# andimarafioti/faster-qwen3-tts

Hardware: AMD Instinct MI355X
Metric: real-time factor (audio s / wall s), Qwen3-TTS-12Hz-0.6B voice-clone streaming chunk_size=8; p50 TTFA in ttfa_ms_p50 (higher is better)
Workload: dtype bf16

## Files before the change

### faster-qwen3-tts_amd/csrc/fq3_api.hip

```cpp
#define FQ3_SKINNY_EXTERN
#include "fq3_ctx.h"
#include "sampler.cuh"
#include "sampler_wave.cuh"
#include "skinny_gemm.cuh"

#include <cstdio>
#include <cstdlib>
#include <cstring>
#include <map>
#include <string>
#include <type_traits>
#include <vector>

using namespace fq3;

static thread_local std::string g_err;
static int fail(int code, const std::string& m) { g_err = m; return code; }
int fq3_fail_(int code, const std::string& m) { return fail(code, m); }
#define HIPCHK(x) do { hipError_t e_ = (x); if (e_ != hipSuccess) return fail(FQ3_EHIP, std::string(#x) + ": " + hipGetErrorString(e_)); } while (0)

extern "C" const char* fq3_last_error(void) { return g_err.c_str(); }
extern "C" void fq3_set_error_(const char* msg) { g_err = msg ? msg : ""; }
extern "C" int fq3_abi_version(void) { return FQ3_ABI_VERSION; }

static int dmalloc(fq3_ctx* c, void** p, size_t bytes, bool zero = true) {
    HIPCHK(hipMalloc(p, bytes));
    if (zero) HIPCHK(hipMemset(*p, 0, bytes));
    c->allocs.push_back(*p);
    return 0;
}
int fq3_dmalloc_(fq3_ctx* c, void** p, size_t bytes) { return dmalloc(c, p, bytes, false); }

static bool dims_ok(const fq3_stack_dims& d) {
    return d.head_dim == kHeadDim && d.hidden % 8 == 0 && d.inter % 8 == 0 && d.n_heads % d.n_kv_heads == 0 &&
           (d.n_heads / d.n_kv_heads == 1 || d.n_heads / d.n_kv_heads == 2 || d.n_heads / d.n_kv_heads == 4) &&
           d.vocab <= kMaxVocab && d.vocab % 8 == 0 && d.hidden <= 2048 && d.inter <= 6144 && d.n_heads * kHeadDim <= 6144 && d.n_layers >= 1;
}

static int cfg_check(const fq3_config* cfg) {
    if (cfg->dtype != FQ3_BF16 && cfg->dtype != FQ3_F32) return fail(FQ3_EINVAL, "dtype must be FQ3_BF16 or FQ3_F32");
    if (!dims_ok(cfg->talker) || !dims_ok(cfg->predictor))
        return fail(FQ3_EUNSUPPORTED, "unsupported dims (need head_dim 128, GQA ratio 1/2/4, vocab <= 4096 and a multiple of 8, "
                                      "hidden <= 2048 and intermediate <= 6144, both multiples of 8)");
    if (cfg->num_code_groups < 2 || cfg->num_code_groups > 64) return fail(FQ3_EINVAL, "num_code_groups");
    if (cfg->max_seq_len < 8) return fail(FQ3_EINVAL, "max_seq_len");
    return 0;
}

static void pool_free_(fq3_kv_pool* p) {
    for (void* q : p->k) if (q) (void)hipFree(q);
    for (void* q : p->v) if (q) (void)hipFree(q);
    delete p;
}

static int pool_create_(const fq3_config* cfg, int n_blocks, fq3_kv_pool** out) {
    if (n_blocks < 1) return fail(FQ3_EINVAL, "fq3_kv_pool_create: n_blocks must be positive");
    fq3_kv_pool* p = new fq3_kv_pool();
    p->dtype = cfg->dtype; p->esz = cfg->dtype == FQ3_BF16 ? 2 : 4;
    p->n_layers = cfg->talker.n_layers; p->n_kv = cfg->talker.n_kv_heads; p->n_blocks = n_blocks;
    p->blk_elems = (size_t)p->n_kv * kKeysPerTile * kHeadDim;
    p->k.assign(p->n_layers, nullptr); p->v.assign(p->n_layers, nullptr);
    const size_t bytes = (size_t)n_blocks * p->blk_elems * p->esz;
    for (int i = 0; i < p->n_layers; ++i) {
        if (hipMalloc(&p->k[i], bytes) != hipSuccess || hipMalloc(&p->v[i], bytes) != hipSuccess ||
            hipMemset(p->k[i], 0, bytes) != hipSuccess || hipMemset(p->v[i], 0, bytes) != hipSuccess) {
            pool_free_(p);
            return fail(FQ3_EHIP, "fq3_kv_pool_create: allocation of " + std::to_string(2 * bytes >> 20) + " MiB per layer failed");
        }
    }
    p->free_list.resize(n_blocks);
    for (int i = 0; i < n_blocks; ++i) p->free_list[i] = n_blocks - 1 - i;
    *out = p;
    return FQ3_OK;
}

extern "C" int fq3_kv_pool_create(const fq3_config* cfg, int n_blocks, fq3_kv_pool** out) {
    if (!cfg || !out) return fail(FQ3_EINVAL, "null argument");
    if (int r = cfg_check(cfg)) return r;
    return pool_create_(cfg, n_blocks, out);
}

extern "C" int fq3_kv_pool_destroy(fq3_kv_pool* p) {
    if (!p) return FQ3_OK;
    if (p->users > 0) return fail(FQ3_ESTATE, "fq3_kv_pool_destroy: contexts are still attached");
    (void)hipDeviceSynchronize();
    pool_free_(p);
    return FQ3_OK;
}

extern "C" int fq3_kv_pool_stats(const fq3_kv_pool* p, int* n_blocks, int* n_free, int* high_water, int64_t* bytes_per_block) {
    if (!p) return fail(FQ3_EINVAL, "null pool");
    fq3_kv_pool* q = const_cast<fq3_kv_pool*>(p);
    std::lock_guard<std::mutex> lk(q->mu);
    if (n_blocks) *n_blocks = p->n_blocks;
    if (n_free) *n_free = (int)p->free_list.size();
    if (high_water) *high_water = p->in_use_high;
    if (bytes_per_block) *bytes_per_block = (int64_t)2 * p->n_layers * p->blk_elems * p->esz;
    return FQ3_OK;
}

struct KvTableVals { int v[128]; };
__global__ void kv_table_write_kernel(int* table, KvTableVals vals, int first, int count) {
    const int i = threadIdx.x;
    if (i < count) table[first + i] = vals.v[i];
}
static void table_write(fq3_ctx* c, const int* ids, int first, int count, hipStream_t s) {
    for (int o = 0; o < count; o += 128) {
        KvTableVals t{};
        const int n = std::min(128, count - o);
        for (int i = 0; i < n; ++i) t.v[i] = ids[o + i];
        hipLaunchKernelGGL(kv_table_write_kernel, dim3(1), dim3(128), 0, s, c->tk.d_table, t, first + o, n);
    }
}

static int kv_ensure(fq3_ctx* c, int n_pos, hipStream_t s, bool sync_copy);
int fq3_kv_ensure_(fq3_ctx* c, int n_pos, hipStream_t s) { return kv_ensure(c, n_pos, s, false); }
static int kv_ensure(fq3_ctx* c, int n_pos, hipStream_t s, bool sync_copy) {
    StackBufs& b = c->tk;
    int need = (std::min(n_pos, b.max_seq) + kKeysPerTile - 1) / kKeysPerTile;
    need = std::min(need, b.max_blocks);
    const int have = (int)b.blocks.size();
    if (need <= have) return 0;
    fq3_kv_pool* p = b.pool;
    {
        std::lock_guard<std::mutex> lk(p->mu);
        if ((int)p->free_list.size() < need - have) {
            char m[200];
            snprintf(m, sizeof m, "KV pool exhausted: %d more block(s) of 64 keys needed, %d free of %d", need - have, (int)p->free_list.size(), p->n_blocks);
            return fail(FQ3_ENOMEM, m);
        }
        for (int i = have; i < need; ++i) { b.blocks.push_back(p->free_list.back()); p->free_list.pop_back(); }
        p->in_use_high = std::max(p->in_use_high, p->n_blocks - (int)p->free_list.size());
    }
    if (sync_copy) HIPCHK(hipMemcpy(b.d_table + have, b.blocks.data() + have, (size_t)(need - have) * sizeof(int), hipMemcpyHostToDevice));
    else table_write(c, b.blocks.data() + have, have, need - have, s);
    return 0;
}

extern "C" int fq3_kv_release(fq3_ctx* c, int keep_positions) {
    if (!c) return fail(FQ3_EINVAL, "null ctx");
    StackBufs& b = c->tk;
    const int keep = std::max(0, std::min((int)b.blocks.size(), (keep_positions + kKeysPerTile - 1) / kKeysPerTile));
    if (keep >= (int)b.blocks.size()) return FQ3_OK;
    std::lock_guard<std::mutex> lk(b.pool->mu);
    while ((int)b.blocks.size() > keep) { b.pool->free_list.push_back(b.blocks.back()); b.blocks.pop_back(); }
    return FQ3_OK;
}

extern "C" int fq3_kv_blocks(const fq3_ctx* c) { return c ? (int)c->tk.blocks.size() : 0; }

extern "C" int fq3_kv_reserve(fq3_ctx* c, int n_positions, void* stream) {
    if (!c) return fail(FQ3_EINVAL, "null ctx");
    if (n_positions < 0) return fail(FQ3_EINVAL, "fq3_kv_reserve: negative position count");
    return fq3_kv_ensure_(c, n_positions, (hipStream_t)stream);
}

static int ctx_build(fq3_ctx* c, const fq3_config* cfg, fq3_kv_pool* pool);
static int ctx_create_(const fq3_config* cfg, fq3_kv_pool* pool, fq3_ctx** out) {
    if (!cfg || !out) return fail(FQ3_EINVAL, "null argument");
    if (int r = cfg_check(cfg)) return r;
    if (pool && (pool->dtype != cfg->dtype || pool->n_layers != cfg->talker.n_layers || pool->n_kv != cfg->talker.n_kv_heads))
        return fail(FQ3_EINVAL, "fq3_ctx_create_pooled: the pool was built for another dtype / layer count / kv head count");
    fq3_ctx* c = new fq3_ctx();
    if (int r = ctx_build(c, cfg, pool)) { const std::string m = g_err; fq3_ctx_destroy(c); g_err = m; return r; }
    *out = c;
    return FQ3_OK;
}
extern "C" int fq3_ctx_create(const fq3_config* cfg, fq3_ctx** out) { return ctx_create_(cfg, nullptr, out); }
extern "C" int fq3_ctx_create_pooled(const fq3_config* cfg, fq3_kv_pool* pool, fq3_ctx** out) {
    if (!pool) return fail(FQ3_EINVAL, "null pool");
    return ctx_create_(cfg, pool, out);
}

static int ctx_build(fq3_ctx* c, const fq3_config* cfg, fq3_kv_pool* pool) {
    c->cfg = *cfg;
    c->esz = cfg->dtype == FQ3_BF16 ? 2 : 4;
    const fq3_stack_dims &t = cfg->talker, &p = cfg->predictor;
    const int pred_seq = cfg->num_code_groups + 1;
    auto alloc_stack = [&](StackBufs& b, const fq3_stack_dims& d, int max_seq) -> int {
        b.max_seq = max_seq;
        b.workers = std::min(kMaxWorkers, (max_seq + kKeysPerTile - 1) / kKeysPerTile);
        b.k.resize(d.n_layers); b.v.resize(d.n_layers);
        const size_t bytes = (size_t)d.n_kv_heads * max_seq * kHeadDim * c->esz;
        for (int i = 0; i < d.n_layers; ++i) {
            if (int r = dmalloc(c, &b.k[i], bytes)) return r;
            if (int r = dmalloc(c, &b.v[i], bytes)) return r;
        }
        return 0;
    };
    int r;
    {
        StackBufs& b = c->tk;
        b.max_seq = cfg->max_seq_len;
        b.max_blocks = (cfg->max_seq_len + kKeysPerTile - 1) / kKeysPerTile;
        b.workers = std::min(kMaxWorkers, b.max_blocks);
        if (!pool) {
            if ((r = pool_create_(cfg, b.max_blocks, &pool))) return r;
            pool->is_private = true;
        }
        b.pool = pool;
        { std::lock_guard<std::mutex> lk(pool->mu); ++pool->users; }
        b.k = pool->k; b.v = pool->v;
        if ((r = dmalloc(c, (void**)&b.d_table, (size_t)b.max_blocks * sizeof(int)))) return r;
        if (pool->is_private && (r = kv_ensure(c, cfg->max_seq_len, nullptr, true))) return r;
    }
    if ((r = alloc_stack(c->pk, p, pred_seq))) return r;
    const int Hm = std::max(t.hidden, p.hidden), Im = std::max(t.inter, p.inter);
    const int qkvm = std::max(t.n_heads + 2 * t.n_kv_heads, p.n_heads + 2 * p.n_kv_heads) * kHeadDim;
    const int Vm = std::max(t.vocab, p.vocab);
    const int G = cfg->num_code_groups;
    const int frames = cfg->max_frames > 0 ? cfg->max_frames : 4096;
    c->cfg.max_frames = frames;
    if ((r = dmalloc(c, &c->h, (size_t)Hm * c->esz))) return r;
    if ((r = dmalloc(c, &c->h2, (size_t)Hm * c->esz))) return r;
    if ((r = dmalloc(c, &c->qkv2, (size_t)qkvm * c->esz))) return r;
    if ((r = dmalloc(c, &c->attn_out, (size_t)qkvm * c->esz))) return r;
    if ((r = dmalloc(c, &c->attn_out2, (size_t)qkvm * c->esz))) return r;
    if ((r = dmalloc(c, &c->act2, (size_t)Im * c->esz))) return r;
    if ((r = dmalloc(c, &c->pred_x2, (size_t)p.hidden * c->esz))) return r;
    if ((r = dmalloc(c, &c->xin, (size_t)Hm * c->esz))) return r;
    if ((r = dmalloc(c, &c->tmp_hidden, (size_t)Hm * c->esz))) return r;
    if ((r = dmalloc(c, &c->qkv, (size_t)qkvm * c->esz))) return r;
    if ((r = dmalloc(c, &c->act, (size_t)Im * c->esz))) return r;
    if ((r = dmalloc(c, &c->logits, (size_t)Vm * c->esz))) return r;
    if ((r = dmalloc(c, &c->past_hidden, (size_t)t.hidden * c->esz))) return r;
    if ((r = dmalloc(c, &c->ph_hold, (size_t)t.hidden * c->esz))) return r;
    if ((r = dmalloc(c, &c->pred_in, (size_t)2 * t.hidden * c->esz))) return r;
    if ((r = dmalloc(c, &c->pred_next, (size_t)t.hidden * c->esz))) return r;
    if ((r = dmalloc(c, &c->pred_x, (size_t)p.hidden * c->esz))) return r;
    if ((r = dmalloc(c, &c->plogits, (size_t)(G - 1) * p.vocab * c->esz))) return r;
    const int maxkv = std::max(t.n_kv_heads, p.n_kv_heads);
    c->part_stride = (size_t)maxkv * kMaxWorkers * 4 * kPartStride;
    if ((r = dmalloc(c, (void**)&c->part, 2 * c->part_stride * sizeof(float)))) return r;
    if ((r = dmalloc(c, (void**)&c->rope_now, 2 * 64 * sizeof(float)))) return r;
    if ((r = dmalloc(c, (void**)&c->seen_api, kMaxVocab))) return r;
    if ((r = dmalloc(c, (void**)&c->st, sizeof(DecodeState)))) return r;
    if ((r = dmalloc(c, (void**)&c->seen, kMaxVocab))) return r;
    if ((r = dmalloc(c, (void**)&c->codes, (size_t)(frames + 1) * G * sizeof(int)))) return r;
    if ((r = dmalloc(c, (void**)&c->ids64, (size_t)64 * sizeof(int64_t)))) return r;
    if ((r = dmalloc(c, (void**)&c->d_pemb, (size_t)64 * sizeof(void*)))) return r;
    HIPCHK(hipStreamCreateWithFlags(&c->cap_stream, hipStreamNonBlocking));
    return FQ3_OK;
}

extern "C" int fq3_set_option(fq3_ctx* c, const char* key, int value) {
    if (!c || !key) return fail(FQ3_EINVAL, "null argument");
    const std::string k(key);
    if (k == "weight_nt") c->opt_nt = value;
    else if (k == "pred_m2") c->opt_m2 = value;
    else if (k == "pred_attn") c->opt_pred_attn = value;
    else if (k == "rows_per_wave_max") c->opt_rmax = value;
    else if (k == "prefill_mode") c->prefill_mode = value;
    else if (k == "flash_prefill") c->opt_flash_prefill = value;
    else if (k == "flash_small") c->opt_flash_small = value;
    else if (k == "swiglu_tile") c->opt_swiglu_tile = value;
    else if (k == "packed_weights") c->opt_packed = value;
    else if (k == "skinny_gemm") c->opt_no_skinny = !value;
    else return fail(FQ3_EINVAL, "unknown option: " + k);
    fq3_graph_reset(c);
    return FQ3_OK;
}

extern "C" int fq3_graph_reset(fq3_ctx* c) {
    if (!c) return fail(FQ3_EINVAL, "null ctx");
    if (c->exec) { (void)hipGraphExecDestroy(c->exec); c->exec = nullptr; }
    if (c->graph) { (void)hipGraphDestroy(c->graph); c->graph = nullptr; }
    return FQ3_OK;
}

namespace {
struct PackedEntry { void* p; int refs; int N, K; };
std::mutex g_packed_mu;
std::map<std::pair<const void*, int>, PackedEntry> g_packed;
}
const void* fq3_packed_find_(const void* W, int kind) {
    std::lock_guard<std::mutex> lk(g_packed_mu);
    auto it = g_packed.find({W, kind});
    return it == g_packed.end() ? nullptr : it->second.p;
}
int fq3_packed_acquire_(const void* W, int N, int K, int kind) {
    if (!W || !skinny_pack_ok(N, K) || (kind == 1 && (N / 2) % 8) || (kind == 2 && N % 512)) return FQ3_EUNSUPPORTED;
    std::lock_guard<std::mutex> lk(g_packed_mu);
    auto it = g_packed.find({W, kind});
    if (it != g_packed.end()) {
        if (it->second.N != N || it->second.K != K) return fail(FQ3_EINVAL, "a matrix is bound with two different shapes");
        ++it->second.refs;
        return FQ3_OK;
    }
    void* p = nullptr;
    if (hipMalloc(&p, (size_t)N * K * 2) != hipSuccess) { (void)hipGetLastError(); return fail(FQ3_ENOMEM, "no device memory for the fragment-major weight copy"); }
    skinny_pack(reinterpret_cast<const bf16_t*>(W), reinterpret_cast<bf16_t*>(p), N, K, kind == 1 ? N / 2 : (kind == 2 ? -(N / 2) : 0), nullptr);
    if (hipStreamSynchronize(nullptr) != hipSuccess) { (void)hipFree(p); return fail(FQ3_EHIP, "packing a weight matrix failed"); }
    g_packed[{W, kind}] = PackedEntry{p, 1, N, K};
    return FQ3_OK;
}
void fq3_packed_release_(const void* W, int kind) {
    std::lock_guard<std::mutex> lk(g_packed_mu);
    auto it = g_packed.find({W, kind});
    if (it == g_packed.end()) return;
    if (--it->second.refs <= 0) { (void)hipFree(it->second.p); g_packed.erase(it); }
}
static void packed_release_all(fq3_ctx* c) {
    for (auto& r : c->packed_refs) fq3_packed_release_(r.first, r.second);
    c->packed_refs.clear();
}
static int packed_acquire_all(fq3_ctx* c) {
    if (c->cfg.dtype != FQ3_BF16) return FQ3_OK;
    auto take = [&](const void* W, int N, int K, int kind) -> int {
        const int r = fq3_packed_acquire_(W, N, K, kind);
        if (r == FQ3_OK) c->packed_refs.emplace_back(W, kind);
        return r == FQ3_EUNSUPPORTED ? FQ3_OK : r;
    };
    auto stack = [&](const std::vector<fq3_layer_weights>& L, const fq3_stack_dims& d) -> int {
        const int qd = d.n_heads * kHeadDim, kvd = d.n_kv_heads * kHeadDim;
        for (const fq3_layer_weights& l : L) {
            if (int r = take(l.qkv, qd + 2 * kvd, d.hidden, 0)) return r;
            if (int r = take(l.o, d.hidden, qd, 0)) return r;
            if (int r = take(l.gate_up, 2 * d.inter, d.hidden, 1)) return r;
            if (int r = take(l.gate_up, 2 * d.inter, d.hidden, 0)) return r;
            if (int r = take(l.down, d.hidden, d.inter, 0)) return r;
        }
        return FQ3_OK;
    };
    if (int r = stack(c->tl, c->cfg.talker)) return r;
    if (int r = stack(c->pl, c->cfg.predictor)) return r;
    for (const fq3_layer_weights& l : c->tl) if (int r = take(l.gate_up, 2 * c->cfg.talker.inter, c->cfg.talker.hidden, 2)) return r;
    if (int r = take(c->wt.codec_head, c->cfg.talker.vocab, c->cfg.talker.hidden, 0)) return r;
    for (const void* h : c->lmh) if (int r = take(h, c->cfg.predictor.vocab, c->cfg.predictor.hidden, 0)) return r;
    return FQ3_OK;
}

extern "C" int fq3_ctx_destroy(fq3_ctx* c) {
    if (!c) return FQ3_OK;
    (void)hipDeviceSynchronize();
    fq3_graph_reset(c);
    packed_release_all(c);
    if (c->cap_stream) (void)hipStreamDestroy(c->cap_stream);
    if (fq3_kv_pool* p = c->tk.pool) {
        (void)fq3_kv_release(c, 0);
        bool last;
        { std::lock_guard<std::mutex> lk(p->mu); last = --p->users == 0; }
        if (p->is_private && last) pool_free_(p);
    }
    for (void* p : c->allocs) (void)hipFree(p);
    delete c;
    return FQ3_OK;
}

extern "C" int fq3_bind_weights(fq3_ctx* c, const fq3_weight_table* w) {
    if (!c || !w) return fail(FQ3_EINVAL, "null argument");
    const int G = c->cfg.num_code_groups;
    if (!w->talker_layers || !w->predictor_layers || !w->codec_embedding || !w->codec_head || !w->talker_final_norm ||
        !w->predictor_final_norm || !w->predictor_embeddings || !w->lm_heads || !w->talker_cos || !w->talker_sin ||
        !w->pred_cos || !w->pred_sin)
        return fail(FQ3_EINVAL, "weight table has null entries");
    if (c->cfg.has_projection && !w->proj_w) return fail(FQ3_EINVAL, "has_projection set but proj_w is null");
    if (w->talker_rope_len < c->cfg.max_seq_len || w->pred_rope_len < G + 1)
        return fail(FQ3_EINVAL, "rope tables shorter than the caches");
    c->wt = *w;
    c->tl.assign(w->talker_layers, w->talker_layers + c->cfg.talker.n_layers);
    c->pl.assign(w->predictor_layers, w->predictor_layers + c->cfg.predictor.n_layers);
    c->pemb.assign(w->predictor_embeddings, w->predictor_embeddings + (G - 1));
    c->lmh.assign(w->lm_heads, w->lm_heads + (G - 1));
    for (auto& l : c->tl) if (!l.qkv || !l.o || !l.gate_up || !l.down || !l.input_norm || !l.post_norm || !l.q_norm || !l.k_norm)
        return fail(FQ3_EINVAL, "talker layer has null weights");
    for (auto& l : c->pl) if (!l.qkv || !l.o || !l.gate_up || !l.down || !l.input_norm || !l.post_norm || !l.q_norm || !l.k_norm)
        return fail(FQ3_EINVAL, "predictor layer has null weights");
    HIPCHK(hipMemcpy(c->d_pemb, c->pemb.data(), (G - 1) * sizeof(void*), hipMemcpyHostToDevice));
    (void)hipDeviceSynchronize();
    packed_release_all(c);
    if (int r = packed_acquire_all(c)) { packed_release_all(c); return r; }
    c->bound = true;
    fq3_graph_reset(c);
    return FQ3_OK;
}

static thread_local int g_rmax = 2;
template <typename T, int NCH, int PRO, int EPI, bool NT, int M = 1>
static void launch_gemv_n(const GemvArgs& a, hipStream_t s) {
    const int rmax = g_rmax;
    int R = (a.N + 1023) / 1024;
    if (R > MaxRows<NCH, EPI>::v) R = MaxRows<NCH, EPI>::v;
    if (rmax > 0 && R > rmax) R = rmax;
    if (R < 1) R = 1;
    const int grid = (a.N + 4 * R - 1) / (4 * R);
    const size_t shm = PRO == PRO_COMBINE ? (size_t)M * a.K * sizeof(float) : 0;
    if constexpr (MaxRows<NCH, EPI>::v >= 2) {
        if (R == 2) { hipLaunchKernelGGL((gemv_kernel<T, NCH, PRO, EPI, NT, M, 2>), dim3(grid), dim3(256), shm, s, a); return; }
    }
    hipLaunchKernelGGL((gemv_kernel<T, NCH, PRO, EPI, NT, M, 1>), dim3(grid), dim3(256), shm, s, a);
}
template <typename T, int PRO, int EPI>
static int launch_gemv2_t(const GemvArgs& a, hipStream_t s) {
    const int need = (a.K + 511) / 512;
    if (need <= 1) launch_gemv_n<T, 1, PRO, EPI, false, 2>(a, s);
    else if (need <= 2) launch_gemv_n<T, 2, PRO, EPI, false, 2>(a, s);
    else if (need <= 4) launch_gemv_n<T, 4, PRO, EPI, false, 2>(a, s);
    else if (PRO != PRO_NORM && need <= 6) { if constexpr (PRO != PRO_NORM) launch_gemv_n<T, 6, PRO, EPI, false, 2>(a, s); }
    else return fail(FQ3_EUNSUPPORTED, PRO == PRO_NORM ? "code predictor hidden size above 2048" : "code predictor GEMV inner dimension above 3072");
    return 0;
}
template <int PRO, int EPI>
static int launch_gemv2(const fq3_ctx* c, const GemvArgs& a, hipStream_t s) {
    g_rmax = c->opt_rmax;
    return c->cfg.dtype == FQ3_BF16 ? launch_gemv2_t<bf16_t, PRO, EPI>(a, s) : launch_gemv2_t<float, PRO, EPI>(a, s);
}
template <typename T, int PRO, int EPI, bool NT>
static int launch_gemv_t(const GemvArgs& a, hipStream_t s) {
    const int need = (a.K + 511) / 512;
    if (need <= 1) launch_gemv_n<T, 1, PRO, EPI, NT>(a, s);
    else if (need <= 2) launch_gemv_n<T, 2, PRO, EPI, NT>(a, s);
    else if (need <= 4) launch_gemv_n<T, 4, PRO, EPI, NT>(a, s);
    else if constexpr (PRO == PRO_NORM) return fail(FQ3_EUNSUPPORTED, "hidden size above 2048");
    else if (need <= 6) launch_gemv_n<T, 6, PRO, EPI, NT>(a, s);
    else if (need <= 12) launch_gemv_n<T, 12, PRO, EPI, NT>(a, s);
    else return fail(FQ3_EUNSUPPORTED, "GEMV inner dimension above 6144");
    return 0;
}
template <int PRO, int EPI>
static int launch_gemv(const fq3_ctx* c, const GemvArgs& a, bool nt, hipStream_t s) {
    g_rmax = c->opt_rmax;
    if (c->cfg.dtype == FQ3_BF16)
        return nt ? launch_gemv_t<bf16_t, PRO, EPI, true>(a, s) : launch_gemv_t<bf16_t, PRO, EPI, false>(a, s);
    return nt ? launch_gemv_t<float, PRO, EPI, true>(a, s) : launch_gemv_t<float, PRO, EPI, false>(a, s);
}

template <typename T, bool PAGED>
static void launch_attn_p(const AttnArgs& a, int rep, int workers, hipStream_t s) {
    dim3 grid(a.n_kv, workers);
    if (rep == 1) hipLaunchKernelGGL((attn_decode_kernel<T, 1, PAGED>), grid, dim3(256), 0, s, a);
    else if (rep == 2) hipLaunchKernelGGL((attn_decode_kernel<T, 2, PAGED>), grid, dim3(256), 0, s, a);
    else hipLaunchKernelGGL((attn_decode_kernel<T, 4, PAGED>), grid, dim3(256), 0, s, a);
}
template <typename T>
static void launch_attn_t(const AttnArgs& a, int rep, int workers, hipStream_t s) {
    if (a.table) launch_attn_p<T, true>(a, rep, workers, s); else launch_attn_p<T, false>(a, rep, workers, s);
}

struct StepSrc { const void* x0; const int* pos_ptr; int pos_imm; bool kv_only_tail = false; };

static int run_stack(fq3_ctx* c, bool talker, const StepSrc& src, hipStream_t s) {
    const fq3_stack_dims& d = talker ? c->cfg.talker : c->cfg.predictor;
    const std::vector<fq3_layer_weights>& L = talker ? c->tl : c->pl;
    StackBufs& kv = talker ? c->tk : c->pk;
    const int rep = d.n_heads / d.n_kv_heads;
    const int q_dim = d.n_heads * kHeadDim, kv_dim = d.n_kv_heads * kHeadDim;
    const bool nt = c->opt_nt == 2 || (c->opt_nt == 1 && talker);
    const float *cos_row, *sin_row;
    if (src.pos_ptr) { cos_row = c->rope_now; sin_row = c->rope_now + 64; }
    else {
        const int rl = talker ? c->wt.talker_rope_len : c->wt.pred_rope_len;
        int rp = src.pos_imm + (talker ? c->rope_delta : 0);
        rp = rp < 0 ? 0 : (rp >= rl ? rl - 1 : rp);
        cos_row = (talker ? c->wt.talker_cos : c->wt.pred_cos) + (size_t)rp * 64;
        sin_row = (talker ? c->wt.talker_sin : c->wt.pred_sin) + (size_t)rp * 64;
    }
    for (int i = 0; i < d.n_layers; ++i) {
        const fq3_layer_weights& w = L[i];
        const void* xin = i == 0 ? src.x0 : c->h;
        GemvArgs g{};
        g.eps = d.rms_eps;
        g.W = w.qkv; g.N = q_dim + 2 * kv_dim; g.K = d.hidden; g.x = xin;
        g.norm_w = w.input_norm; g.y = c->qkv;
        if (int r = launch_gemv<PRO_NORM, EPI_STORE>(c, g, nt, s)) return r;
        const bool tail_skip = src.kv_only_tail && i == d.n_layers - 1;
        GemvArgs o{};
        o.W = w.o; o.N = d.hidden; o.K = q_dim; o.y = c->h; o.res = xin; o.rep = rep;
        AttnArgs a{};
        a.qkv = c->qkv; a.q_norm_w = w.q_norm; a.k_norm_w = w.k_norm; a.eps = d.rms_eps;
        a.cos_row = cos_row; a.sin_row = sin_row;
        a.kcache = kv.k[i]; a.vcache = kv.v[i]; a.max_seq = kv.max_seq;
        a.table = kv.d_table; a.blk_stride = kv.pool ? (int)kv.pool->blk_elems : 0;
        a.pos_ptr = src.pos_ptr; a.pos_imm = src.pos_imm;
        a.done_ptr = src.pos_ptr ? &c->st->done : nullptr;
        a.n_pad = talker ? c->n_pad : 0;
        a.n_kv = d.n_kv_heads; a.part = c->part;
        a.scale = 1.0f / sqrtf((float)kHeadDim);
        a.rep = rep; a.out = c->attn_out;
        const bool pred_attn = c->opt_pred_attn && !talker && !src.pos_ptr && src.pos_imm <= 16;
        if (pred_attn) {
            if (c->cfg.dtype == FQ3_BF16) hipLaunchKernelGGL((attn_pred_kernel<bf16_t>), dim3(d.n_heads), dim3(64), 0, s, a);
            else hipLaunchKernelGGL((attn_pred_kernel<float>), dim3(d.n_heads), dim3(64), 0, s, a);
            if (tail_skip) break;
            o.x = c->attn_out;
            if (int r = launch_gemv<PRO_PLAIN, EPI_RESIDUAL>(c, o, nt, s)) return r;
        } else {
            if (c->cfg.dtype == FQ3_BF16) launch_attn_t<bf16_t>(a, rep, kv.workers, s);
            else launch_attn_t<float>(a, rep, kv.workers, s);
            if (tail_skip) break;
            o.part = c->part; o.n_part = kv.workers;
            if (int r = launch_gemv<PRO_COMBINE, EPI_RESIDUAL>(c, o, nt, s)) return r;
        }
        GemvArgs m{};
        m.eps = d.rms_eps; m.W = w.gate_up; m.N = d.inter; m.K = d.hidden; m.x = c->h;
        m.norm_w = w.post_norm; m.y = c->act; m.up_off = d.inter;
        if (int r = launch_gemv<PRO_NORM, EPI_SWIGLU>(c, m, nt, s)) return r;
        GemvArgs dn{};
        dn.W = w.down; dn.N = d.hidden; dn.K = d.inter; dn.x = c->act; dn.y = c->h; dn.res = c->h;
        if (int r = launch_gemv<PRO_PLAIN, EPI_RESIDUAL>(c, dn, nt, s)) return r;
    }
    return 0;
}

static int run_predictor_pair(fq3_ctx* c, const void* x_a, const void* x_b, hipStream_t s) {
    const fq3_stack_dims& d = c->cfg.predictor;
    StackBufs& kv = c->pk;
    const int rep = d.n_heads / d.n_kv_heads;
    const int q_dim = d.n_heads * kHeadDim, kv_dim = d.n_kv_heads * kHeadDim;
    for (int i = 0; i < d.n_layers; ++i) {
        const fq3_layer_weights& w = c->pl[i];
        const void* xa = i == 0 ? x_a : c->h;
        const void* xb = i == 0 ? x_b : c->h2;
        GemvArgs g{};
        g.eps = d.rms_eps; g.W = w.qkv; g.N = q_dim + 2 * kv_dim; g.K = d.hidden; g.x = xa; g.x2 = xb;
        g.norm_w = w.input_norm; g.y = c->qkv; g.y2 = c->qkv2;
        if (int r = launch_gemv2<PRO_NORM, EPI_STORE>(c, g, s)) return r;
        for (int m = 0; m < 2; ++m) {
            AttnArgs a{};
            a.qkv = m == 0 ? c->qkv : c->qkv2; a.q_norm_w = w.q_norm; a.k_norm_w = w.k_norm; a.eps = d.rms_eps;
            a.cos_row = c->wt.pred_cos + (size_t)m * 64; a.sin_row = c->wt.pred_sin + (size_t)m * 64;
            a.kcache = kv.k[i]; a.vcache = kv.v[i]; a.max_seq = kv.max_seq;
            a.pos_ptr = nullptr; a.pos_imm = m; a.n_pad = 0; a.n_kv = d.n_kv_heads;
            a.part = c->part + (size_t)m * c->part_stride; a.scale = 1.0f / sqrtf((float)kHeadDim);
            a.rep = rep; a.out = m == 0 ? c->attn_out : c->attn_out2;
            if (c->opt_pred_attn) {
                if (c->cfg.dtype == FQ3_BF16) hipLaunchKernelGGL((attn_pred_kernel<bf16_t>), dim3(d.n_heads), dim3(64), 0, s, a);
                else hipLaunchKernelGGL((attn_pred_kernel<float>), dim3(d.n_heads), dim3(64), 0, s, a);
            } else if (c->cfg.dtype == FQ3_BF16) launch_attn_t<bf16_t>(a, rep, kv.workers, s);
            else launch_attn_t<float>(a, rep, kv.workers, s);
        }
        GemvArgs o{};
        o.W = w.o; o.N = d.hidden; o.K = q_dim; o.y = c->h; o.y2 = c->h2; o.res = xa; o.res2 = xb; o.rep = rep;
        if (c->opt_pred_attn) {
            o.x = c->attn_out; o.x2 = c->attn_out2;
            if (int r = launch_gemv2<PRO_PLAIN, EPI_RESIDUAL>(c, o, s)) return r;
        } else {
            o.part = c->part; o.part_stride2 = c->part_stride; o.n_part = kv.workers;
            if (int r = launch_gemv2<PRO_COMBINE, EPI_RESIDUAL>(c, o, s)) return r;
        }
        GemvArgs m{};
        m.eps = d.rms_eps; m.W = w.gate_up; m.N = d.inter; m.K = d.hidden; m.x = c->h; m.x2 = c->h2;
        m.norm_w = w.post_norm; m.y = c->act; m.y2 = c->act2; m.up_off = d.inter;
        if (int r = launch_gemv2<PRO_NORM, EPI_SWIGLU>(c, m, s)) return r;
        GemvArgs dn{};
        dn.W = w.down; dn.N = d.hidden; dn.K = d.inter; dn.x = c->act; dn.x2 = c->act2; dn.y = c->h; dn.y2 = c->h2;
        dn.res = c->h; dn.res2 = c->h2;
        if (int r = launch_gemv2<PRO_PLAIN, EPI_RESIDUAL>(c, dn, s)) return r;
    }
    return 0;
}

#define NEED_BOUND(c) do { if (!(c)) return fail(FQ3_EINVAL, "null ctx"); if (!(c)->bound) return fail(FQ3_ESTATE, "weights not bound"); } while (0)
#define LAUNCH_CHECK() HIPCHK(hipGetLastError())

extern "C" int fq3_set_generation_state(fq3_ctx* c, int n_pad, int rope_delta) {
    if (!c) return fail(FQ3_EINVAL, "null ctx");
    if (n_pad < 0 || n_pad >= c->cfg.max_seq_len) return fail(FQ3_EINVAL, "n_pad out of range");
    if (c->n_pad != n_pad || c->rope_delta != rope_delta) fq3_graph_reset(c);
    c->n_pad = n_pad; c->rope_delta = rope_delta;
    return FQ3_OK;
}

template <typename T, bool TO_CACHE>
__global__ __launch_bounds__(256) void kv_paged_copy_kernel(T* cache, const int* table, int blk_stride, T* dense, int n_kv, int L) {
    constexpr int EPC = 16 / (int)sizeof(T), CPR = kHeadDim / EPC;
    const int i = blockIdx.x * 256 + threadIdx.x;
    if (i >= n_kv * L * CPR) return;
    const int ch = i % CPR, row = i / CPR, key = row % L, h = row / L;
    T* cp = cache + (size_t)table[key / kKeysPerTile] * blk_stride + ((size_t)h * kKeysPerTile + key % kKeysPerTile) * kHeadDim + ch * EPC;
    T* dp = dense + ((size_t)h * L + key) * kHeadDim + ch * EPC;
    if (TO_CACHE) *reinterpret_cast<u32x4*>(cp) = *reinterpret_cast<const u32x4*>(dp);
    else *reinterpret_cast<u32x4*>(dp) = *reinterpret_cast<const u32x4*>(cp);
}
template <typename T, bool TO_CACHE>
static void kv_paged_copy(fq3_ctx* c, int layer, void* k, void* v, int L, hipStream_t s) {
    const int nk = c->cfg.talker.n_kv_heads, n = nk * L * (kHeadDim * (int)sizeof(T) / 16);
    if (n <= 0) return;
    const int bs = (int)c->tk.pool->blk_elems;
    hipLaunchKernelGGL((kv_paged_copy_kernel<T, TO_CACHE>), dim3((n + 255) / 256), dim3(256), 0, s, (T*)c->tk.k[layer], c->tk.d_table, bs, (T*)k, nk, L);
    hipLaunchKernelGGL((kv_paged_copy_kernel<T, TO_CACHE>), dim3((n + 255) / 256), dim3(256), 0, s, (T*)c->tk.v[layer], c->tk.d_table, bs, (T*)v, nk, L);
}

extern "C" int fq3_kv_import(fq3_ctx* c, int layer, const void* k, const void* v, int L, void* stream) {
    if (!c || !k || !v) return fail(FQ3_EINVAL, "null argument");
    if (layer < 0 || layer >= c->cfg.talker.n_layers) return fail(FQ3_EINVAL, "layer out of range");
    if (L > c->cfg.max_seq_len) {
        char b[256];
        snprintf(b, sizeof b, "Input is too long: prefill has %d tokens but max_seq_len=%d. Use shorter text or shorter reference audio.",
                 L, c->cfg.max_seq_len);
        return fail(FQ3_ETOOLONG, b);
    }
    hipStream_t s = (hipStream_t)stream;
    if (int r = fq3_kv_ensure_(c, L, s)) return r;
    if (c->cfg.dtype == FQ3_BF16) kv_paged_copy<bf16_t, true>(c, layer, const_cast<void*>(k), const_cast<void*>(v), L, s);
    else kv_paged_copy<float, true>(c, layer, const_cast<void*>(k), const_cast<void*>(v), L, s);
    LAUNCH_CHECK();
    return FQ3_OK;
}

extern "C" int fq3_kv_export(fq3_ctx* c, int layer, void* k, void* v, int L, void* stream) {
    if (!c || !k || !v) return fail(FQ3_EINVAL, "null argument");
    if (layer < 0 || layer >= c->cfg.talker.n_layers || L > c->cfg.max_seq_len) return fail(FQ3_EINVAL, "range");
    if (L > (int)c->tk.blocks.size() * kKeysPerTile) return fail(FQ3_EINVAL, "fq3_kv_export: rows beyond the blocks this context owns");
    hipStream_t s = (hipStream_t)stream;
    if (c->cfg.dtype == FQ3_BF16) kv_paged_copy<bf16_t, false>(c, layer, k, v, L, s);
    else kv_paged_copy<float, false>(c, layer, k, v, L, s);
    LAUNCH_CHECK();
    return FQ3_OK;
}

struct KvAdoptTab { void* dst[128]; const void* src[128]; };
template <typename T>
__global__ __launch_bounds__(256) void kv_adopt_kernel(KvAdoptTab t, const int* dst_table, const int* src_table, int blk_elems) {
    const int which = blockIdx.x, b = blockIdx.y;
    const u32x4* s = reinterpret_cast<const u32x4*>(reinterpret_cast<const T*>(t.src[which]) + (size_t)src_table[b] * blk_elems);
    u32x4* d = reinterpret_cast<u32x4*>(reinterpret_cast<T*>(t.dst[which]) + (size_t)dst_table[b] * blk_elems);
    const int n16 = blk_elems * (int)sizeof(T) / 16;
    for (int i = threadIdx.x; i < n16; i += 256) d[i] = s[i];
}

extern "C" int fq3_kv_adopt(fq3_ctx* dst, fq3_ctx* src, int L, void* stream) {
    if (!dst || !src) return fail(FQ3_EINVAL, "null ctx");
    if (dst == src) return fail(FQ3_EINVAL, "fq3_kv_adopt: source and destination are the same context");
    const auto &a = dst->cfg, &b = src->cfg;
    if (a.dtype != b.dtype || a.talker.n_layers != b.talker.n_layers || a.talker.n_kv_heads != b.talker.n_kv_heads)
        return fail(FQ3_EINVAL, "fq3_kv_adopt: contexts of different shape");
    if (L < 0 || L > src->tk.max_seq || L > (int)src->tk.blocks.size() * kKeysPerTile) return fail(FQ3_EINVAL, "fq3_kv_adopt: L outside the source cache");
    if (L > dst->tk.max_seq) {
        char m[256];
        snprintf(m, sizeof m, "Input is too long: prefill has %d tokens but max_seq_len=%d. Use shorter text or shorter reference audio.", L, a.max_seq_len);
        return fail(FQ3_ETOOLONG, m);
    }
    const int nl = a.talker.n_layers;
    if (2 * nl > 128) return fail(FQ3_EUNSUPPORTED, "fq3_kv_adopt: more than 64 layers");
    if (L == 0) return FQ3_OK;
    hipStream_t s = (hipStream_t)stream;
    const int nb = (L + kKeysPerTile - 1) / kKeysPerTile;
    if (dst->tk.pool == src->tk.pool) {
        (void)fq3_kv_release(dst, 0);
        const size_t take = std::min(src->tk.blocks.size(), (size_t)dst->tk.max_blocks);
        dst->tk.blocks.assign(src->tk.blocks.begin(), src->tk.blocks.begin() + take);
        if (take < src->tk.blocks.size()) {
            std::lock_guard<std::mutex> lk(src->tk.pool->mu);
            for (size_t i = take; i < src->tk.blocks.size(); ++i) src->tk.pool->free_list.push_back(src->tk.blocks[i]);
        }
        src->tk.blocks.clear();
        table_write(dst, dst->tk.blocks.data(), 0, (int)take, s);
        LAUNCH_CHECK();
        return FQ3_OK;
    }
    if (int r = fq3_kv_ensure_(dst, L, s)) return r;
    KvAdoptTab t{};
    for (int l = 0; l < nl; ++l) { t.dst[2 * l] = dst->tk.k[l]; t.src[2 * l] = src->tk.k[l]; t.dst[2 * l + 1] = dst->tk.v[l]; t.src[2 * l + 1] = src->tk.v[l]; }
    const dim3 grid(2 * nl, nb);
    const int be = (int)dst->tk.pool->blk_elems;
    if (a.dtype == FQ3_BF16) hipLaunchKernelGGL((kv_adopt_kernel<bf16_t>), grid, dim3(256), 0, s, t, dst->tk.d_table, src->tk.d_table, be);
    else hipLaunchKernelGGL((kv_adopt_kernel<float>), grid, dim3(256), 0, s, t, dst->tk.d_table, src->tk.d_table, be);
    LAUNCH_CHECK();
    return FQ3_OK;
}

static int final_norm(fq3_ctx* c, bool talker, const void* x, void* y, hipStream_t s) {
    const fq3_stack_dims& d = talker ? c->cfg.talker : c->cfg.predictor;
    const void* w = talker ? c->wt.talker_final_norm : c->wt.predictor_final_norm;
    if (c->cfg.dtype == FQ3_BF16)
        hipLaunchKernelGGL((rmsnorm_kernel<bf16_t>), dim3(1), dim3(256), 0, s, (const bf16_t*)x, (const bf16_t*)w, (bf16_t*)y, d.hidden, d.rms_eps);
    else
        hipLaunchKernelGGL((rmsnorm_kernel<float>), dim3(1), dim3(256), 0, s, (const float*)x, (const float*)w, (float*)y, d.hidden, d.rms_eps);
    return 0;
}

extern "C" int fq3_talker_step(fq3_ctx* c, const void* embeds, int position, void* out_hidden, void* stream) {
    NEED_BOUND(c);
    if (!embeds || !out_hidden) return fail(FQ3_EINVAL, "null argument");
    if (position < 0 || position >= c->cfg.max_seq_len) return fail(FQ3_EINVAL, "position outside the static cache");
    hipStream_t s = (hipStream_t)stream;
    if (int r = fq3_kv_ensure_(c, position + 1, s)) return r;
    StepSrc src{embeds, nullptr, position};
    if (int r = run_stack(c, true, src, s)) return r;
    final_norm(c, true, c->h, out_hidden, s);
    LAUNCH_CHECK();
    return FQ3_OK;
}

extern "C" int fq3_codec_head(fq3_ctx* c, const void* hidden, void* out_logits, void* stream) {
    NEED_BOUND(c);
    if (!hidden || !out_logits) return fail(FQ3_EINVAL, "null argument");
    GemvArgs g{};
    g.W = c->wt.codec_head; g.N = c->cfg.talker.vocab; g.K = c->cfg.talker.hidden; g.x = hidden; g.y = out_logits;
    if (int r = launch_gemv<PRO_PLAIN, EPI_STORE>(c, g, true, (hipStream_t)stream)) return r;
    LAUNCH_CHECK();
    return FQ3_OK;
}

extern "C" int fq3_prefill(fq3_ctx* c, const void* embeds, int L, int n_pad, void* out_logits, void* out_hidden,
                           void* stream) {
    NEED_BOUND(c);
    if (!embeds || L <= 0) return fail(FQ3_EINVAL, "bad prompt");
    if (L > c->cfg.max_seq_len) {
        char b[256];
        snprintf(b, sizeof b, "Input is too long: prefill has %d tokens but max_seq_len=%d. Use shorter text or shorter reference audio.",
                 L, c->cfg.max_seq_len);
        return fail(FQ3_ETOOLONG, b);
    }
    if (n_pad < 0 || n_pad >= L) return fail(FQ3_EINVAL, "n_pad");
    if (int r = fq3_set_generation_state(c, n_pad, -n_pad)) return r;
    hipStream_t s = (hipStream_t)stream;
    if (int r = fq3_kv_ensure_(c, L, s)) return r;
    void* hid = out_hidden ? out_hidden : c->tmp_hidden;
    if (c->prefill_mode != 1 && L - n_pad >= 4) {
        if (int r = fq3_prefill_mfma_(c, embeds, L, n_pad, out_logits, hid, s)) return r;
        LAUNCH_CHECK();
        return FQ3_OK;
    }
    const size_t rowb = (size_t)c->cfg.talker.hidden * c->esz;
    for (int i = n_pad; i < L; ++i) {
        StepSrc src{(const char*)embeds + rowb * i, nullptr, i};
        if (int r = run_stack(c, true, src, s)) return r;
    }
    final_norm(c, true, c->h, hid, s);
    if (out_logits) {
        GemvArgs g{};
        g.W = c->wt.codec_head; g.N = c->cfg.talker.vocab; g.K = c->cfg.talker.hidden; g.x = hid; g.y = out_logits;
        if (int r = launch_gemv<PRO_PLAIN, EPI_STORE>(c, g, true, s)) return r;
    }
    LAUNCH_CHECK();
    return FQ3_OK;
}

extern "C" int fq3_prefill_reserve(fq3_ctx* c) {
    NEED_BOUND(c);
    return fq3_prefill_reserve_(c);
}

extern "C" int fq3_prefill_batch(fq3_ctx* const* ctxs, int n, const void* const* embeds, const int* L, const int* n_pad,
                                 void* const* out_logits, void* const* out_hidden, void* stream) {
    if (!ctxs || !embeds || !L || !n_pad || !out_hidden || n < 1 || n > 64) return fail(FQ3_EINVAL, "fq3_prefill_batch: bad argument");
    long total = 0;
    bool packed = true;
    for (int q = 0; q < n; ++q) {
        fq3_ctx* c = ctxs[q];
        NEED_BOUND(c);
        if (!embeds[q] || !out_hidden[q] || L[q] <= 0) return fail(FQ3_EINVAL, "fq3_prefill_batch: bad prompt");
        if (L[q] > c->cfg.max_seq_len) {
            char b[256];
            snprintf(b, sizeof b, "Input is too long: prefill has %d tokens but max_seq_len=%d. Use shorter text or shorter reference audio.",
                     L[q], c->cfg.max_seq_len);
            return fail(FQ3_ETOOLONG, b);
        }
        if (n_pad[q] < 0 || n_pad[q] >= L[q]) return fail(FQ3_EINVAL, "n_pad");
        total += L[q];
        const fq3_ctx* c0 = ctxs[0];
        packed = packed && c->cfg.dtype == c0->cfg.dtype && c->wt.codec_head == c0->wt.codec_head && c->tl.size() == c0->tl.size() &&
                 !c->tl.empty() && c->tl[0].qkv == c0->tl[0].qkv && c->prefill_mode != 1 && L[q] - n_pad[q] >= 4;
        for (int p = 0; p < q; ++p) if (ctxs[p] == c) return fail(FQ3_EINVAL, "fq3_prefill_batch: a context appears twice");
    }
    packed = packed && n > 1 && total <= ctxs[0]->cfg.max_seq_len;
    if (!packed) {
        for (int q = 0; q < n; ++q)
            if (int r = fq3_prefill(ctxs[q], embeds[q], L[q], n_pad[q], out_logits ? out_logits[q] : nullptr, out_hidden[q], stream)) return r;
        return FQ3_OK;
    }
    for (int q = 0; q < n; ++q)
        if (int r = fq3_set_generation_state(ctxs[q], n_pad[q], -n_pad[q])) return r;
    {
        std::vector<int> had(n);
        for (int q = 0; q < n; ++q) had[q] = (int)ctxs[q]->tk.blocks.size();
        for (int q = 0; q < n; ++q)
            if (int r = fq3_kv_ensure_(ctxs[q], L[q], (hipStream_t)stream)) {
                const std::string m = g_err;
                for (int p = 0; p < q; ++p) (void)fq3_kv_release(ctxs[p], had[p] * kKeysPerTile);
                g_err = m;
                return r;
            }
    }
    if (int r = fq3_prefill_batch_mfma_(ctxs, n, embeds, L, n_pad, out_logits, out_hidden, (hipStream_t)stream)) return r;
    LAUNCH_CHECK();
    return FQ3_OK;
}

int fq3_codec_head_launch_(fq3_ctx* c, const void* hidden, void* out_logits, hipStream_t s) {
    GemvArgs g{};
    g.W = c->wt.codec_head; g.N = c->cfg.talker.vocab; g.K = c->cfg.talker.hidden; g.x = hidden; g.y = out_logits;
    return launch_gemv<PRO_PLAIN, EPI_STORE>(c, g, true, s);
}

extern "C" int fq3_set_prefill_mode(fq3_ctx* c, int mode) { return fq3_set_option(c, "prefill_mode", mode); }

__global__ void build_seen_kernel(const int64_t* history, int n, unsigned char* seen, int V) {
    for (int i = threadIdx.x; i < V; i += blockDim.x) seen[i] = 0;
    __syncthreads();
    for (int i = threadIdx.x; i < n; i += blockDim.x) { const int id = (int)history[i]; if (id >= 0 && id < V) seen[id] = 1; }
}
template <typename F>
static void dispatch_nc(int V, F&& f) {
    if (V <= 2048) f(std::integral_constant<int, 1>{});
    else f(std::integral_constant<int, 2>{});
}

template <typename T>
static void launch_sample_pred(const DecodeState* st, const T* lg, int V, int cb, const SampleCfg& cfg, const T* nz,
                               int* codes, int G, int64_t* out64, const T* next_emb, T* next_in, int H, bool wave,
                               const TeacherForcing* tf, hipStream_t s) {
    if (wave) dispatch_nc(V, [&](auto nc) {
        constexpr int NC = decltype(nc)::value;
        hipLaunchKernelGGL((sample_pred_wave_kernel<T, NC>), dim3(1), dim3(256), 0, s, st, lg, V, cb, cfg, nz, codes, G,
                           out64, next_emb, next_in, H, tf);
    });
    else hipLaunchKernelGGL((sample_pred_kernel<T>), dim3(1), dim3(256), 0, s, st, lg, V, cb, cfg, nz, codes, G, out64,
                            next_emb, next_in, H, tf);
}
template <typename T>
static void launch_sample_talker(DecodeState* st, const T* lg, int V, const unsigned char* seen, int G, bool wave,
                                 const TeacherForcing* tf, hipStream_t s) {
    if (wave) dispatch_nc(V, [&](auto nc) {
        constexpr int NC = decltype(nc)::value;
        hipLaunchKernelGGL((sample_talker_wave_kernel<T, NC>), dim3(1), dim3(256), 0, s, st, lg, V, seen, G, tf);
    });
    else hipLaunchKernelGGL((sample_talker_kernel<T>), dim3(1), dim3(256), 0, s, st, lg, V, seen, G, tf);
}
template <typename T>
static void launch_sample_api(fq3_ctx* c, const T* lg, int V, const SampleCfg& cfg, const int64_t* history, int n_hist,
                              const T* noise, int64_t* out, hipStream_t s) {
    if (cfg.top_p >= 1.0f) {
        const unsigned char* seen = nullptr;
        if (n_hist > 0) {
            hipLaunchKernelGGL(build_seen_kernel, dim3(1), dim3(256), 0, s, history, n_hist, c->seen_api, V);
            seen = c->seen_api;
        }
        dispatch_nc(V, [&](auto nc) {
            constexpr int NC = decltype(nc)::value;
            hipLaunchKernelGGL((sample_api_wave_kernel<T, NC>), dim3(1), dim3(256), 0, s, lg, V, cfg, seen, noise, out);
        });
    } else {
        hipLaunchKernelGGL((sample_api_kernel<T>), dim3(1), dim3(256), 0, s, lg, V, cfg, history, n_hist, noise, out);
    }
}

static SampleCfg to_cfg(const fq3_sampling& s) {
    SampleCfg c{};
    c.temperature = s.temperature; c.top_k = s.top_k; c.top_p = s.top_p; c.do_sample = s.do_sample;
    c.rep_penalty = s.repetition_penalty; c.sup_lo = 0; c.sup_hi = 0; c.keep_id = -1; c.sup_extra = -1;
    return c;
}

extern "C" int fq3_sample(fq3_ctx* c, const void* logits, int V, const fq3_sampling* sp, const int64_t* history,
                          int n_hist, int sup_lo, int sup_hi, int keep_id, int suppress_eos, const void* noise,
                          int64_t* out_token, void* stream) {
    if (!c || !logits || !sp || !out_token) return fail(FQ3_EINVAL, "null argument");
    if (V <= 0 || V > kMaxVocab || V % 8) return fail(FQ3_EUNSUPPORTED, "vocab must be a multiple of 8 and at most 4096");
    if (sp->do_sample && !noise) return fail(FQ3_EINVAL, "do_sample needs a noise vector");
    if (sp->do_sample && !(sp->temperature > 0.f)) return fail(FQ3_EINVAL, "temperature must be > 0");
    SampleCfg cfg = to_cfg(*sp);
    cfg.sup_lo = sup_lo; cfg.sup_hi = sup_hi; cfg.keep_id = keep_id;
    cfg.sup_extra = suppress_eos ? c->cfg.codec_eos_token_id : -1;
    hipStream_t s = (hipStream_t)stream;
    if (c->cfg.dtype == FQ3_BF16)
        launch_sample_api<bf16_t>(c, (const bf16_t*)logits, V, cfg, history, history ? n_hist : 0, (const bf16_t*)noise, out_token, s);
    else
        launch_sample_api<float>(c, (const float*)logits, V, cfg, history, history ? n_hist : 0, (const float*)noise, out_token, s);
    LAUNCH_CHECK();
    return FQ3_OK;
}

template <typename T>
__global__ __launch_bounds__(256) void rep_penalty_kernel(T* logits, int V, const unsigned char* seen, float penalty) {
    for (int i = threadIdx.x; i < V; i += 256) {
        if (!seen[i]) continue;
        const float v = DT<T>::ld(logits + i);
        DT<T>::st(logits + i, v > 0.f ? v / penalty : v * penalty);
    }
}
extern "C" int fq3_apply_repetition_penalty(fq3_ctx* c, void* logits, int V, const int64_t* history, int n_hist,
                                            float penalty, void* stream) {
    if (!c || !logits) return fail(FQ3_EINVAL, "null argument");
    if (V <= 0 || V > kMaxVocab) return fail(FQ3_EUNSUPPORTED, "vocab must be at most 4096");
    if (penalty == 1.0f || n_hist <= 0 || !history) return FQ3_OK;
    hipStream_t s = (hipStream_t)stream;
    hipLaunchKernelGGL(build_seen_kernel, dim3(1), dim3(256), 0, s, history, n_hist, c->seen_api, V);
    if (c->cfg.dtype == FQ3_BF16) hipLaunchKernelGGL((rep_penalty_kernel<bf16_t>), dim3(1), dim3(256), 0, s, (bf16_t*)logits, V, c->seen_api, penalty);
    else hipLaunchKernelGGL((rep_penalty_kernel<float>), dim3(1), dim3(256), 0, s, (float*)logits, V, c->seen_api, penalty);
    LAUNCH_CHECK();
    return FQ3_OK;
}

extern "C" int fq3_set_predictor_sampling(fq3_ctx* c, const fq3_sampling* s) {
    if (!c || !s) return fail(FQ3_EINVAL, "null argument");
    if (s->do_sample && !(s->temperature > 0.f)) return fail(FQ3_EINVAL, "temperature must be > 0");
    if ((s->top_p >= 1.0f) != (c->pred_sampling.top_p >= 1.0f)) fq3_graph_reset(c);
    c->pred_sampling = *s;
    return FQ3_OK;
}

template <typename T>
static int predictor_passes_t(fq3_ctx* c, const DecodeState* st_dev, const void* pred_input, const void* noise_imm,
                              int64_t* out64, void* out_logits, hipStream_t s) {
    const fq3_stack_dims &p = c->cfg.predictor, &t = c->cfg.talker;
    const int G = c->cfg.num_code_groups, Vp = p.vocab, Ht = t.hidden;
    SampleCfg scfg = to_cfg(c->pred_sampling);
    for (int pass = 0; pass < G; ++pass) {
        const void* hsrc = c->h;
        if (pass == 0 && c->opt_m2) {
            const T* xa = (const T*)pred_input;
            const T* xb = (const T*)pred_input + Ht;
            if (c->cfg.has_projection) {
                GemvArgs g{};
                g.W = c->wt.proj_w; g.bias = c->wt.proj_b; g.N = p.hidden; g.K = Ht; g.x = xa; g.x2 = xb; g.y = c->pred_x; g.y2 = c->pred_x2;
                if (int r = launch_gemv2<PRO_PLAIN, EPI_STORE>(c, g, s)) return r;
                xa = (const T*)c->pred_x; xb = (const T*)c->pred_x2;
            }
            if (int r = run_predictor_pair(c, xa, xb, s)) return r;
            pass = 1;
            hsrc = c->h2;
        } else {
        const T* x_talker = pass < 2 ? (const T*)pred_input + (size_t)pass * Ht : (const T*)c->pred_next;
        const void* x0 = x_talker;
        if (c->cfg.has_projection) {
            GemvArgs g{};
            g.W = c->wt.proj_w; g.bias = c->wt.proj_b; g.N = p.hidden; g.K = Ht; g.x = x_talker; g.y = c->pred_x;
            if (int r = launch_gemv<PRO_PLAIN, EPI_STORE>(c, g, false, s)) return r;
            x0 = c->pred_x;
        }
        StepSrc src{x0, nullptr, pass};
        src.kv_only_tail = pass == 0;
        if (int r = run_stack(c, false, src, s)) return r;
        }
        if (pass == 0) continue;
        const int cb = pass - 1;
        T* lg = out_logits ? (T*)out_logits + (size_t)cb * Vp : (T*)c->plogits + (size_t)cb * Vp;
        GemvArgs hgm{};
        hgm.eps = p.rms_eps; hgm.W = c->lmh[cb]; hgm.N = Vp; hgm.K = p.hidden; hgm.x = hsrc;
        hgm.norm_w = c->wt.predictor_final_norm; hgm.y = lg;
        if (int r = launch_gemv<PRO_NORM, EPI_STORE>(c, hgm, false, s)) return r;
        const T* nz = noise_imm ? (const T*)noise_imm + (size_t)cb * Vp : nullptr;
        const T* next_emb = cb + 1 < G - 1 ? (const T*)c->pemb[cb] : nullptr;
        launch_sample_pred<T>(st_dev, (const T*)lg, Vp, cb, scfg, nz, st_dev ? c->codes : nullptr, G, out64, next_emb,
                              (T*)c->pred_next, Ht, c->pred_sampling.top_p >= 1.0f, st_dev ? c->tf : nullptr, s);
    }
    return 0;
}

extern "C" int fq3_predictor_loop(fq3_ctx* c, const void* pred_input, const void* noise, int64_t* out_ids,
                                  void* out_logits, void* stream) {
    NEED_BOUND(c);
    if (!pred_input || !out_ids) return fail(FQ3_EINVAL, "null argument");
    if (c->pred_sampling.do_sample && !noise) return fail(FQ3_EINVAL, "predictor sampling enabled but no noise given");
    hipStream_t s = (hipStream_t)stream;
    int r = c->cfg.dtype == FQ3_BF16 ? predictor_passes_t<bf16_t>(c, nullptr, pred_input, noise, out_ids, out_logits, s)
                                     : predictor_passes_t<float>(c, nullptr, pred_input, noise, out_ids, out_logits, s);
    if (r) return r;
    LAUNCH_CHECK();
    return FQ3_OK;
}

__global__ __launch_bounds__(256) void decode_arm_kernel(DecodeState* st, DecodeState init, unsigned char* seen, int seen_bytes,
                                                         uint32_t* past_hidden, const uint32_t* ph_src, int ph_words) {
    for (int i = threadIdx.x; i < seen_bytes / 4; i += 256) reinterpret_cast<uint32_t*>(seen)[i] = 0u;
    for (int i = threadIdx.x; i < ph_words; i += 256) past_hidden[i] = ph_src[i];
    if (threadIdx.x == 0) *st = init;
}
__global__ void decode_set_forced_kernel(TeacherForcing* tf, const int* forced, int* decisions) {
    tf->forced = forced; tf->decisions = decisions;
}

extern "C" int fq3_decode_begin(fq3_ctx* c, const fq3_decode_params* p, void* stream) {
    NEED_BOUND(c);
    if (!p || !p->past_hidden || !p->tts_pad_embed) return fail(FQ3_EINVAL, "null argument");
    if (p->trailing_len > 0 && !p->trailing_text) return fail(FQ3_EINVAL, "trailing_text");
    if (p->talker.do_sample && (!p->talker_noise || p->noise_frames <= 0)) return fail(FQ3_EINVAL, "talker sampling needs a noise ring");
    if (c->pred_sampling.do_sample && (!p->pred_noise || p->noise_frames <= 0)) return fail(FQ3_EINVAL, "predictor sampling needs a noise ring");
    if (p->talker.do_sample && !(p->talker.temperature > 0.f)) return fail(FQ3_EINVAL, "temperature must be > 0");
    if (p->max_new_tokens > c->cfg.max_frames) return fail(FQ3_EINVAL, "max_new_tokens exceeds the context's max_frames");
    if (p->prefill_len <= 0 || p->prefill_len > c->cfg.max_seq_len) return fail(FQ3_EINVAL, "prefill_len");
    if (p->first_token < 0 || p->first_token >= c->cfg.talker.vocab) return fail(FQ3_EINVAL, "first_token outside the codec vocabulary");
    if (p->gen_step < 0 || p->min_new_tokens < 0 || p->max_new_tokens < 0) return fail(FQ3_EINVAL, "negative counters");
    const bool wave = p->talker.top_p >= 1.0f;
    if (wave != c->talker_wave) { fq3_graph_reset(c); c->talker_wave = wave; }
    hipStream_t s = (hipStream_t)stream;
    if (int r = fq3_kv_ensure_(c, p->prefill_len + p->max_new_tokens + 1, s)) return r;
    DecodeState h{};
    h.token = p->first_token; h.frame = 0; h.pos = p->prefill_len; h.gen_step = p->gen_step; h.done = 0; h.text_open = 0;
    h.min_new = p->min_new_tokens; h.max_new = p->max_new_tokens; h.trailing_len = p->trailing_len;
    h.noise_frames = p->noise_frames > 0 ? p->noise_frames : 1;
    h.eos_id = c->cfg.codec_eos_token_id; h.max_seq = c->cfg.max_seq_len;
    h.n_pad = c->n_pad; h.rope_delta = c->rope_delta;
    h.sup_lo = c->cfg.talker.vocab - 1024 > 0 ? c->cfg.talker.vocab - 1024 : 0; h.sup_hi = c->cfg.talker.vocab;
    h.t_temperature = p->talker.temperature; h.t_top_k = p->talker.top_k; h.t_top_p = p->talker.top_p;
    h.t_do_sample = p->talker.do_sample; h.t_rep_penalty = p->talker.repetition_penalty;
    h.p_temperature = c->pred_sampling.temperature; h.p_top_k = c->pred_sampling.top_k; h.p_top_p = c->pred_sampling.top_p;
    h.p_do_sample = c->pred_sampling.do_sample;
    h.trailing_text = p->trailing_text; h.tts_pad = p->tts_pad_embed; h.talker_noise = p->talker_noise; h.pred_noise = p->pred_noise;
    hipLaunchKernelGGL(decode_arm_kernel, dim3(1), dim3(256), 0, s, c->st, h, c->seen, (int)kMaxVocab,
                       (uint32_t*)c->past_hidden, (const uint32_t*)p->past_hidden, (int)((size_t)c->cfg.talker.hidden * c->esz / 4));
    LAUNCH_CHECK();
    c->armed = true; c->tt_open = false; c->tt_session = false; c->tt_rows = 0; c->tt_cap = 0;
    c->begin_trailing = p->trailing_text; c->begin_trailing_len = p->trailing_len > 0 ? p->trailing_len : 0;
    return FQ3_OK;
}

__global__ void decode_cancel_kernel(DecodeState* st) { st->done = 1; }
extern "C" int fq3_decode_cancel(fq3_ctx* c, void* stream) {
    if (!c) return fail(FQ3_EINVAL, "null ctx");
    hipLaunchKernelGGL(decode_cancel_kernel, dim3(1), dim3(1), 0, (hipStream_t)stream, c->st);
    LAUNCH_CHECK();
    return FQ3_OK;
}

extern "C" int fq3_decode_set_forced(fq3_ctx* c, const int32_t* forced_codes, int32_t* decisions, void* stream) {
    NEED_BOUND(c);
    if (!c->tf) {
        if (!forced_codes && !decisions) return FQ3_OK;
        if (int r = dmalloc(c, (void**)&c->tf, sizeof(TeacherForcing))) return r;
        fq3_graph_reset(c);
    }
    hipLaunchKernelGGL(decode_set_forced_kernel, dim3(1), dim3(1), 0, (hipStream_t)stream, c->tf, forced_codes, decisions);
    LAUNCH_CHECK();
    return FQ3_OK;
}

template <typename T>
static int enqueue_frame_t(fq3_ctx* c, hipStream_t s) {
    const fq3_stack_dims& t = c->cfg.talker;
    const int G = c->cfg.num_code_groups, H = t.hidden;
    DecodeState* st = c->st;
    hipLaunchKernelGGL((frame_begin_kernel<T>), dim3(1), dim3(256), 0, s, st, (const T*)c->wt.codec_embedding,
                       (const T*)c->past_hidden, (T*)c->ph_hold, (T*)c->pred_in, c->codes, c->seen, H, G);
    if (int r = predictor_passes_t<T>(c, st, c->pred_in, nullptr, nullptr, nullptr, s)) return r;
    EmbTables tabs{};
    tabs.t[0] = c->wt.codec_embedding;
    for (int i = 1; i < G; ++i) tabs.t[i] = c->pemb[i - 1];
    if (G != 16) return fail(FQ3_EUNSUPPORTED, "the fused loop is built for 16 code groups");
    hipLaunchKernelGGL((embed_sum_kernel<T, 16>), dim3(1), dim3(256), 0, s, st, tabs, c->codes, (T*)c->xin, H,
                       c->wt.talker_cos, c->wt.talker_sin, c->wt.talker_rope_len, c->rope_delta, c->rope_now);
    StepSrc src{c->xin, &st->pos, 0};
    if (int r = run_stack(c, true, src, s)) return r;
    GemvArgs g{};
    g.eps = t.rms_eps; g.W = c->wt.codec_head; g.N = t.vocab; g.K = H; g.x = c->h;
    g.norm_w = c->wt.talker_final_norm; g.y = c->logits; g.xn_out = c->past_hidden;
    if (int r = launch_gemv<PRO_NORM, EPI_STORE>(c, g, true, s)) return r;
    launch_sample_talker<T>(st, (const T*)c->logits, t.vocab, c->seen, G, c->talker_wave, c->tf, s);
    return 0;
}
static int enqueue_frame(fq3_ctx* c, hipStream_t s) {
    return c->cfg.dtype == FQ3_BF16 ? enqueue_frame_t<bf16_t>(c, s) : enqueue_frame_t<float>(c, s);
}

extern "C" int fq3_graph_capture(fq3_ctx* c, void* stream) {
    NEED_BOUND(c);
    if (c->exec) return FQ3_OK;
    (void)stream;
    hipStream_t cs = c->cap_stream;
    HIPCHK(hipStreamBeginCapture(cs, hipStreamCaptureModeRelaxed));
    int r = enqueue_frame(c, cs);
    hipGraph_t g = nullptr;
    hipError_t e = hipStreamEndCapture(cs, &g);
    if (r) { if (g) (void)hipGraphDestroy(g); return r; }
    if (e != hipSuccess) return fail(FQ3_EHIP, std::string("hipStreamEndCapture: ") + hipGetErrorString(e));
    c->graph = g;
    HIPCHK(hipGraphInstantiate(&c->exec, c->graph, nullptr, nullptr, 0));
    return FQ3_OK;
}

extern "C" int fq3_decode_frames(fq3_ctx* c, int n_frames, void* stream) {
    NEED_BOUND(c);
    hipStream_t s = (hipStream_t)stream;
    for (int i = 0; i < n_frames; ++i) {
        if (c->exec) { HIPCHK(hipGraphLaunch(c->exec, s)); }
        else if (int r = enqueue_frame(c, s)) return r;
    }
    LAUNCH_CHECK();
    return FQ3_OK;
}

extern "C" int fq3_decode_poll(fq3_ctx* c, int* n_frames_total, int* done, void* stream) {
    if (!c) return fail(FQ3_EINVAL, "null ctx");
    hipStream_t s = (hipStream_t)stream;
    DecodeState h;
    HIPCHK(hipMemcpyAsync(&h, c->st, sizeof h, hipMemcpyDeviceToHost, s));
    HIPCHK(hipStreamSynchronize(s));
    if (n_frames_total) *n_frames_total = h.frame;
    if (done) *done = h.done == 2 ? 2 : (h.done || h.token == h.eos_id);
    return FQ3_OK;
}

__global__ void codes_to_i64_kernel(const int* src, int64_t* dst, int n) {
    const int i = blockIdx.x * blockDim.x + threadIdx.x;
    if (i < n) dst[i] = src[i];
}

extern "C" int fq3_decode_codes(fq3_ctx* c, int from, int count, int64_t* out, void* stream) {
    if (!c || !out) return fail(FQ3_EINVAL, "null argument");
    if (from < 0 || count < 0 || from + count > c->cfg.max_frames) return fail(FQ3_EINVAL, "range");
    const int G = c->cfg.num_code_groups, n = count * G;
    if (n == 0) return FQ3_OK;
    hipLaunchKernelGGL(codes_to_i64_kernel, dim3((n + 255) / 256), dim3(256), 0, (hipStream_t)stream,
                       c->codes + (size_t)from * G, out, n);
    LAUNCH_CHECK();
    return FQ3_OK;
}
```

### faster-qwen3-tts_amd/csrc/fq3_ctx.h

```cpp
#pragma once
#include "../../include/fq3hip.h"
#include "decode_kernels.cuh"
#include <hip/hip_runtime.h>
#include <mutex>
#include <string>
#include <utility>
#include <vector>

struct fq3_kv_pool {
    int dtype = 0, esz = 2, n_layers = 0, n_kv = 0, n_blocks = 0;
    size_t blk_elems = 0;
    std::vector<void*> k, v;
    std::vector<int> free_list;
    std::mutex mu;
    int in_use_high = 0;
    int users = 0;
    bool is_private = false;
};

struct StackBufs {
    std::vector<void*> k, v;
    int max_seq = 0, workers = 1;
    fq3_kv_pool* pool = nullptr;
    int* d_table = nullptr;
    std::vector<int> blocks;
    int max_blocks = 0;
};

struct fq3_ctx {
    fq3_config cfg{};
    int esz = 2;
    std::vector<fq3_layer_weights> tl, pl;
    fq3_weight_table wt{};
    std::vector<const void*> pemb, lmh;
    const void** d_pemb = nullptr;
    bool bound = false;
    StackBufs tk, pk;
    void *h = nullptr, *xin = nullptr, *qkv = nullptr, *act = nullptr, *logits = nullptr, *past_hidden = nullptr;
    void *pred_in = nullptr, *pred_x = nullptr, *pred_next = nullptr, *plogits = nullptr, *tmp_hidden = nullptr;
    void *attn_out = nullptr, *attn_out2 = nullptr;
    void *h2 = nullptr, *qkv2 = nullptr, *act2 = nullptr, *pred_x2 = nullptr;
    size_t part_stride = 0;
    float* part = nullptr;
    float* rope_now = nullptr;
    unsigned char* seen_api = nullptr;
    fq3::DecodeState* st = nullptr;
    fq3::TeacherForcing* tf = nullptr;
    unsigned char* seen = nullptr;
    int* codes = nullptr;
    int64_t* ids64 = nullptr;
    int n_pad = 0, rope_delta = 0;
    int opt_nt = 1;
    int opt_m2 = 1;
    int opt_pred_attn = 1;
    int opt_rmax = 2;
    int opt_flash_prefill = 1;
    int opt_flash_small = 1;
    int opt_swiglu_tile = 1;
    int opt_packed = 1;
    std::vector<std::pair<const void*, int>> packed_refs;
    int opt_no_skinny = 0;
    int prefill_mode = 0;
    bool talker_wave = true;
    fq3_sampling pred_sampling{0.9f, 50, 1.0f, 1, 1.0f};
    hipGraph_t graph = nullptr;
    hipGraphExec_t exec = nullptr;
    hipStream_t cap_stream = nullptr;
    std::vector<void*> allocs;
    fq3_prompt_weights pw{};
    bool pw_bound = false;
    void *pw_x = nullptr, *pw_h = nullptr;
    int pw_cap = 0;
    void* ph_hold = nullptr;
    void *tt_tab = nullptr, *tt_x = nullptr, *tt_h = nullptr;
    int tt_alloc = 0;
    int tt_cap = 0, tt_rows = 0;
    bool tt_open = false, tt_session = false;
    bool armed = false;
    const void* begin_trailing = nullptr; int begin_trailing_len = 0;
    void *pf_x = nullptr, *pf_xn = nullptr, *pf_qkv = nullptr, *pf_att = nullptr, *pf_gu = nullptr, *pf_act = nullptr, *pf_ws = nullptr;
};


const void* fq3_packed_find_(const void* W, int kind);
int fq3_packed_acquire_(const void* W, int N, int K, int kind);
void fq3_packed_release_(const void* W, int kind);

int fq3_fail_(int code, const std::string& m);
int fq3_kv_ensure_(fq3_ctx* c, int n_pos, hipStream_t s);
int fq3_prefill_reserve_(fq3_ctx* c);
int fq3_prefill_mfma_(fq3_ctx* c, const void* embeds, int L, int n_pad, void* out_logits, void* out_hidden, hipStream_t s);
int fq3_prefill_batch_mfma_(fq3_ctx* const* cs, int n, const void* const* embeds, const int* L, const int* n_pad, void* const* out_logits,
                            void* const* out_hidden, hipStream_t s);
int fq3_codec_head_launch_(fq3_ctx* c, const void* hidden, void* out_logits, hipStream_t s);
int fq3_dmalloc_(fq3_ctx* c, void** p, size_t bytes);
void fq3_text_project_launch_(fq3_ctx* c, const int64_t* ids, int n, void* x, void* h, void* out, hipStream_t s);
```

### faster-qwen3-tts_amd/csrc/sampler.cuh

```cuda
#pragma once
#include "fq3_common.cuh"
#include "decode_kernels.cuh"

namespace fq3 {

constexpr int kMaxVocab = 4096;

__device__ __forceinline__ uint32_t okey(float f) {
    const uint32_t u = __float_as_uint(f);
    return (u & 0x80000000u) ? ~u : (u | 0x80000000u);
}

struct ArgMax { float v; int i; };
__device__ __forceinline__ ArgMax amax2(ArgMax a, ArgMax b) {
    return (b.v > a.v || (b.v == a.v && b.i < a.i)) ? b : a;
}
__device__ __forceinline__ int block_argmax(ArgMax a, float* redv, int* redi) {
#pragma unroll
    for (int o = 32; o > 0; o >>= 1) {
        ArgMax b; b.v = __shfl_xor(a.v, o, 64); b.i = __shfl_xor(a.i, o, 64);
        a = amax2(a, b);
    }
    const int w = threadIdx.x >> 6;
    __syncthreads();
    if ((threadIdx.x & 63) == 0) { redv[w] = a.v; redi[w] = a.i; }
    __syncthreads();
    ArgMax r; r.v = redv[0]; r.i = redi[0];
    for (int i = 1; i < 4; ++i) { ArgMax b; b.v = redv[i]; b.i = redi[i]; r = amax2(r, b); }
    return r.i;
}

struct SampleCfg {
    float temperature; int top_k; float top_p; int do_sample; float rep_penalty;
    int sup_lo, sup_hi, keep_id, sup_extra;
};

struct SampleSmem {
    float vals[kMaxVocab];
    unsigned long long keys[kMaxVocab];
    int hist[256];
    float redv[8]; int redi[8];
    int sel_bin, sel_k;
};

template <typename T>
__device__ int sample_core(SampleSmem& sm, int V, const SampleCfg& c, const unsigned char* seen, const T* noise) {
    const int tid = threadIdx.x;
    for (int i = tid; i < V; i += 256) {
        float x = sm.vals[i];
        if (seen && c.rep_penalty != 1.0f && seen[i])
            x = x > 0.f ? DT<T>::rnd(x / c.rep_penalty) : DT<T>::rnd(x * c.rep_penalty);
        if ((i >= c.sup_lo && i < c.sup_hi && i != c.keep_id) || i == c.sup_extra) x = -INFINITY;
        sm.vals[i] = x;
    }
    __syncthreads();
    if (!c.do_sample) {
        ArgMax a; a.v = -INFINITY; a.i = 0x7fffffff;
        for (int i = tid; i < V; i += 256) { ArgMax b; b.v = sm.vals[i]; b.i = i; a = amax2(a, b); }
        return block_argmax(a, sm.redv, sm.redi);
    }
    for (int i = tid; i < V; i += 256) sm.vals[i] = DT<T>::rnd(sm.vals[i] / c.temperature);
    __syncthreads();
    if (c.top_k > 0) {
        int kk = min(c.top_k, V);
        uint32_t prefix = 0, mask = 0;
        constexpr int kPasses = sizeof(T) == 2 ? 2 : 4;
        for (int pass = 0; pass < kPasses; ++pass) {
            const int shift = 24 - 8 * pass;
            sm.hist[tid] = 0;
            __syncthreads();
            for (int i = tid; i < V; i += 256) {
                const uint32_t k = okey(sm.vals[i]);
                if ((k & mask) == prefix) atomicAdd(&sm.hist[(k >> shift) & 255], 1);
            }
            __syncthreads();
            int cnt = sm.hist[tid];
            int incl = cnt;
            {
                const int lane = tid & 63, w = tid >> 6;
#pragma unroll
                for (int o = 1; o < 64; o <<= 1) {
                    const int t = __shfl_down(incl, o, 64);
                    if (lane + o < 64) incl += t;
                }
                __syncthreads();
                if (lane == 0) sm.redi[w] = incl;
                __syncthreads();
                for (int ww = w + 1; ww < 4; ++ww) incl += sm.redi[ww];
            }
            const int excl = incl - cnt;
            if (excl < kk && kk <= incl) { sm.sel_bin = tid; sm.sel_k = kk - excl; }
            __syncthreads();
            prefix |= ((uint32_t)sm.sel_bin) << shift;
            mask |= 0xFFu << shift;
            kk = sm.sel_k;
            __syncthreads();
        }
        const uint32_t kth = prefix;
        for (int i = tid; i < V; i += 256)
            if ((okey(sm.vals[i]) & mask) < kth) sm.vals[i] = -INFINITY;
        __syncthreads();
    }
    if (c.top_p < 1.0f) {
        int n = 1;
        while (n < V) n <<= 1;
        for (int i = tid; i < n; i += 256)
            sm.keys[i] = i < V ? (((unsigned long long)(~okey(sm.vals[i]))) << 32) | (unsigned)i : ~0ull;
        __syncthreads();
        for (int k = 2; k <= n; k <<= 1)
            for (int j = k >> 1; j > 0; j >>= 1) {
                for (int i = tid; i < n; i += 256) {
                    const int p = i ^ j;
                    if (p > i) {
                        const unsigned long long A = sm.keys[i], B = sm.keys[p];
                        const bool up = (i & k) == 0;
                        if ((A > B) == up) { sm.keys[i] = B; sm.keys[p] = A; }
                    }
                }
                __syncthreads();
            }
        float mx = -INFINITY;
        for (int i = tid; i < V; i += 256) mx = fmaxf(mx, sm.vals[i]);
        mx = block_max<4>(mx, sm.redv);
        float se = 0.f;
        for (int i = tid; i < V; i += 256) se += expf(sm.vals[i] - mx);
        se = block_sum<4>(se, sm.redv);
        if (tid == 0) {
            const float thr = DT<T>::rnd(c.top_p);
            float cum = 0.f;
            for (int j = 0; j < V; ++j) {
                const int idx = (int)(sm.keys[j] & 0xffffffffu);
                const float x = sm.vals[idx];
                if (x == -INFINITY) break;
                const float p = DT<T>::rnd(expf(x - mx) / se);
                cum += p;
                if (j > 0 && DT<T>::rnd(cum) > thr) sm.vals[idx] = -INFINITY;
            }
        }
        __syncthreads();
    }
    float mx = -INFINITY;
    for (int i = tid; i < V; i += 256) mx = fmaxf(mx, sm.vals[i]);
    mx = block_max<4>(mx, sm.redv);
    float se = 0.f;
    for (int i = tid; i < V; i += 256) se += expf(sm.vals[i] - mx);
    se = block_sum<4>(se, sm.redv);
    ArgMax a; a.v = -INFINITY; a.i = 0x7fffffff;
    for (int i = tid; i < V; i += 256) {
        const float p = DT<T>::rnd(expf(sm.vals[i] - mx) / se);
        ArgMax b; b.v = DT<T>::rnd(p / DT<T>::ld(noise + i)); b.i = i;
        a = amax2(a, b);
    }
    return block_argmax(a, sm.redv, sm.redi);
}

template <typename T>
__global__ __launch_bounds__(256) void sample_api_kernel(const T* logits, int V, SampleCfg c, const int64_t* history,
                                                         int n_hist, const T* noise, int64_t* out) {
    __shared__ SampleSmem sm;
    __shared__ unsigned char seen_l[kMaxVocab];
    for (int i = threadIdx.x; i < V; i += 256) { sm.vals[i] = DT<T>::ld(logits + i); seen_l[i] = 0; }
    __syncthreads();
    for (int i = threadIdx.x; i < n_hist; i += 256) { const int id = (int)history[i]; if (id >= 0 && id < V) seen_l[id] = 1; }
    __syncthreads();
    const int tok = sample_core<T>(sm, V, c, n_hist > 0 ? seen_l : nullptr, noise);
    if (threadIdx.x == 0) out[0] = tok;
}

template <typename T>
__global__ __launch_bounds__(256) void sample_pred_kernel(const DecodeState* st, const T* logits, int V, int cb,
                                                          SampleCfg c_imm, const T* noise_imm, int* codes, int G,
                                                          int64_t* out64, const T* next_emb, T* next_in, int H, const TeacherForcing* tf) {
    if (st && st->done) return;
    __shared__ SampleSmem sm;
    __shared__ int s_tok;
    SampleCfg c = c_imm;
    const T* noise = noise_imm;
    int frame = 0;
    if (st) {
        c.temperature = st->p_temperature; c.top_k = st->p_top_k; c.top_p = st->p_top_p; c.do_sample = st->p_do_sample;
        frame = st->frame;
        if (st->pred_noise)
            noise = gptr(reinterpret_cast<const T*>(st->pred_noise)) + ((size_t)(frame % st->noise_frames) * (G - 1) + cb) * V;
    }
    for (int i = threadIdx.x; i < V; i += 256) sm.vals[i] = DT<T>::ld(logits + i);
    __syncthreads();
    int tok = sample_core<T>(sm, V, c, nullptr, noise);
    if (st) tok = forced_or(tf, frame * G + 1 + cb, tok);
    if (threadIdx.x == 0) {
        if (codes) codes[(size_t)frame * G + 1 + cb] = tok;
        if (out64) out64[cb] = tok;
    }
    if (next_emb)
        for (int e = threadIdx.x; e < H; e += 256) next_in[e] = next_emb[(size_t)tok * H + e];
}

template <typename T>
__global__ __launch_bounds__(256) void sample_talker_kernel(DecodeState* st, const T* logits, int V,
                                                            const unsigned char* seen, int G, const TeacherForcing* tf) {
    if (st->done) return;
    __shared__ SampleSmem sm;
    SampleCfg c;
    c.temperature = st->t_temperature; c.top_k = st->t_top_k; c.top_p = st->t_top_p; c.do_sample = st->t_do_sample;
    c.rep_penalty = st->t_rep_penalty;
    c.sup_lo = st->sup_lo; c.sup_hi = st->sup_hi; c.keep_id = st->eos_id;
    const int frame = st->frame;
    c.sup_extra = (frame + 1 < st->min_new) ? st->eos_id : -1;
    const T* noise = st->talker_noise
        ? gptr(reinterpret_cast<const T*>(st->talker_noise)) + (size_t)(frame % st->noise_frames) * V : nullptr;
    for (int i = threadIdx.x; i < V; i += 256) sm.vals[i] = DT<T>::ld(logits + i);
    __syncthreads();
    int tok = sample_core<T>(sm, V, c, seen, noise);
    __syncthreads();
    tok = forced_or(tf, (frame + 1) * G, tok);
    if (threadIdx.x == 0) {
        st->token = tok; st->frame = frame + 1; st->pos += 1; st->gen_step += 1;
    }
}

}
```

### faster-qwen3-tts_amd/csrc/sampler_wave.cuh

```cuda
#pragma once
#include "sampler.cuh"

namespace fq3 {

__device__ __forceinline__ ArgMax wave_argmax(ArgMax a) {
    ArgMax r;
    r.v = wave_max(a.v);
    r.i = wave_min_i32(a.v == r.v ? a.i : 0x7fffffff);
    return r;
}

struct BlkSmem { int cnt[2][4]; float f[4]; float av[4]; int ai[4]; };

__device__ __forceinline__ float blk_max4(float v, BlkSmem& sm) {
    v = wave_max(v);
    __syncthreads();
    if ((threadIdx.x & 63) == 0) sm.f[threadIdx.x >> 6] = v;
    __syncthreads();
    return fmaxf(fmaxf(sm.f[0], sm.f[1]), fmaxf(sm.f[2], sm.f[3]));
}
__device__ __forceinline__ float blk_sum4(float v, BlkSmem& sm) {
    v = wave_sum(v);
    __syncthreads();
    if ((threadIdx.x & 63) == 0) sm.f[threadIdx.x >> 6] = v;
    __syncthreads();
    return (sm.f[0] + sm.f[1]) + (sm.f[2] + sm.f[3]);
}
__device__ __forceinline__ int blk_argmax4(ArgMax a, BlkSmem& sm) {
    a = wave_argmax(a);
    __syncthreads();
    if ((threadIdx.x & 63) == 0) { sm.av[threadIdx.x >> 6] = a.v; sm.ai[threadIdx.x >> 6] = a.i; }
    __syncthreads();
    ArgMax r; r.v = sm.av[0]; r.i = sm.ai[0];
#pragma unroll
    for (int i = 1; i < 4; ++i) { ArgMax b; b.v = sm.av[i]; b.i = sm.ai[i]; r = amax2(r, b); }
    return r.i;
}

template <typename T, int NC>
__device__ int sample_wave_core(Raw8<T> (&xraw)[NC], int V, const SampleCfg& c, const unsigned char* seen,
                                const T* noise, BlkSmem& sm) {
    const int tid = threadIdx.x;
    float x[NC][8];
    Raw8<T> nz[NC];
    const bool samp = c.do_sample != 0;
#pragma unroll
    for (int j = 0; j < NC; ++j) {
        const int off = j * 2048 + tid * 8;
        if (samp && off < V) ldraw<false>(nz[j], noise + off); else zero(nz[j]);
    }
    const bool pen = seen && c.rep_penalty != 1.0f;
#pragma unroll
    for (int j = 0; j < NC; ++j) {
        const int off = j * 2048 + tid * 8;
        unpack(xraw[j], x[j]);
        unsigned long long sb = 0ull;
        if (pen && off < V) sb = *reinterpret_cast<const unsigned long long*>(seen + off);
#pragma unroll
        for (int i = 0; i < 8; ++i) {
            const int id = off + i;
            float v = x[j][i];
            if (pen && ((sb >> (8 * i)) & 0xffull)) v = v > 0.f ? DT<T>::rnd(v / c.rep_penalty) : DT<T>::rnd(v * c.rep_penalty);
            if (id >= V || (id >= c.sup_lo && id < c.sup_hi && id != c.keep_id) || id == c.sup_extra) v = -INFINITY;
            x[j][i] = v;
        }
    }
    if (!samp) {
        ArgMax a; a.v = -INFINITY; a.i = 0x7fffffff;
#pragma unroll
        for (int j = 0; j < NC; ++j)
#pragma unroll
            for (int i = 0; i < 8; ++i) { ArgMax b; b.v = x[j][i]; b.i = j * 2048 + tid * 8 + i; a = amax2(a, b); }
        return blk_argmax4(a, sm);
    }
#pragma unroll
    for (int j = 0; j < NC; ++j)
#pragma unroll
        for (int i = 0; i < 8; ++i) x[j][i] = DT<T>::rnd(x[j][i] / c.temperature);
    if (c.top_k > 0) {
        const int kk = min(c.top_k, V);
        uint32_t key[NC][8];
#pragma unroll
        for (int j = 0; j < NC; ++j)
#pragma unroll
            for (int i = 0; i < 8; ++i) key[j][i] = (j * 2048 + tid * 8 + i) < V ? okey(x[j][i]) : 0u;
        uint32_t prefix = 0;
        constexpr int kLowBit = sizeof(T) == 2 ? 16 : 0;
        const int wave = tid >> 6;
#pragma unroll 1
        for (int bit = 31; bit >= kLowBit; --bit) {
            const uint32_t cand = prefix | (1u << bit);
            int cnt = 0;
#pragma unroll
            for (int j = 0; j < NC; ++j)
#pragma unroll
                for (int i = 0; i < 8; ++i) cnt += __popcll(__ballot(key[j][i] >= cand));
            int* slot = sm.cnt[bit & 1];
            if ((tid & 63) == 0) slot[wave] = cnt;
            __syncthreads();
            const int tot = (slot[0] + slot[1]) + (slot[2] + slot[3]);
            if (tot >= kk) prefix = cand;
            if (tot == kk) break;
        }
#pragma unroll
        for (int j = 0; j < NC; ++j)
#pragma unroll
            for (int i = 0; i < 8; ++i)
                if (key[j][i] < prefix) x[j][i] = -INFINITY;
    }
    float mx = -INFINITY;
#pragma unroll
    for (int j = 0; j < NC; ++j)
#pragma unroll
        for (int i = 0; i < 8; ++i) mx = fmaxf(mx, x[j][i]);
    mx = blk_max4(mx, sm);
    float se = 0.f;
#pragma unroll
    for (int j = 0; j < NC; ++j)
#pragma unroll
        for (int i = 0; i < 8; ++i) { x[j][i] = expf(x[j][i] - mx); se += x[j][i]; }
    se = blk_sum4(se, sm);
    ArgMax a; a.v = -INFINITY; a.i = 0x7fffffff;
#pragma unroll
    for (int j = 0; j < NC; ++j) {
        float q[8];
        unpack(nz[j], q);
#pragma unroll
        for (int i = 0; i < 8; ++i) {
            const int id = j * 2048 + tid * 8 + i;
            const float p = DT<T>::rnd(x[j][i] / se);
            ArgMax b; b.v = id < V ? DT<T>::rnd(p / q[i]) : -INFINITY; b.i = id;
            a = amax2(a, b);
        }
    }
    return blk_argmax4(a, sm);
}

template <typename T, int NC>
__device__ __forceinline__ void issue_logits(Raw8<T> (&xraw)[NC], const T* logits, int V) {
#pragma unroll
    for (int j = 0; j < NC; ++j) {
        const int off = j * 2048 + threadIdx.x * 8;
        if (off < V) ldraw<false>(xraw[j], logits + off); else zero(xraw[j]);
    }
}

template <typename T, int NC>
__global__ __launch_bounds__(256) void sample_api_wave_kernel(const T* logits, int V, SampleCfg c, const unsigned char* seen,
                                                             const T* noise, int64_t* out) {
    __shared__ BlkSmem sm;
    Raw8<T> xraw[NC];
    issue_logits<T, NC>(xraw, logits, V);
    const int tok = sample_wave_core<T, NC>(xraw, V, c, seen, noise, sm);
    if (threadIdx.x == 0) out[0] = tok;
}

template <typename T, int NC>
__device__ __forceinline__ int sample_nucleus_from_regs(Raw8<T> (&xraw)[NC], int V, const SampleCfg& c, const unsigned char* seen,
                                                        const T* noise, SampleSmem& big) {
#pragma unroll
    for (int j = 0; j < NC; ++j) {
        float f[8];
        unpack(xraw[j], f);
#pragma unroll
        for (int i = 0; i < 8; ++i) {
            const int id = j * 2048 + threadIdx.x * 8 + i;
            if (id < V) big.vals[id] = f[i];
        }
    }
    __syncthreads();
    const int tok = sample_core<T>(big, V, c, seen, noise);
    __syncthreads();
    return tok;
}

template <typename T, int NC, bool NUCLEUS = false>
__device__ __forceinline__ void sample_pred_wave_body(const DecodeState* st, const T* logits, int V, int cb,
                                                      const SampleCfg& c_imm, const T* noise_imm, int* codes, int G,
                                                      int64_t* out64, const T* next_emb, T* next_in, int H, const TeacherForcing* tf = nullptr) {
    __shared__ BlkSmem sm;
    Raw8<T> xraw[NC];
    issue_logits<T, NC>(xraw, logits, V);
    SampleCfg c = c_imm;
    const T* noise = noise_imm;
    int frame = 0;
    if (st) {
        if (st->done) return;
        c.temperature = st->p_temperature; c.top_k = st->p_top_k; c.top_p = st->p_top_p; c.do_sample = st->p_do_sample;
        frame = st->frame;
        if (st->pred_noise)
            noise = gptr(reinterpret_cast<const T*>(st->pred_noise)) + ((size_t)(frame % st->noise_frames) * (G - 1) + cb) * V;
    }
    int tok;
    if constexpr (NUCLEUS) {
        __shared__ SampleSmem big;
        if (c.do_sample && c.top_p < 1.0f) tok = sample_nucleus_from_regs<T, NC>(xraw, V, c, nullptr, noise, big);
        else tok = sample_wave_core<T, NC>(xraw, V, c, nullptr, noise, sm);
    } else {
        tok = sample_wave_core<T, NC>(xraw, V, c, nullptr, noise, sm);
    }
    if (st) tok = forced_or(tf, frame * G + 1 + cb, tok);
    if (threadIdx.x == 0) {
        if (codes) codes[(size_t)frame * G + 1 + cb] = tok;
        if (out64) out64[cb] = tok;
    }
    if (next_emb) {
        const T* src = next_emb + (size_t)tok * H;
        for (int e = threadIdx.x * 8; e < H; e += 256 * 8) {
            Raw8<T> r; ldraw<false>(r, src + e);
            if (sizeof(T) == 2) *reinterpret_cast<u32x4*>(reinterpret_cast<char*>(next_in) + (size_t)e * 2) = *reinterpret_cast<u32x4*>(&r);
            else { float f[8]; unpack(r, f);
#pragma unroll
                   for (int i = 0; i < 8; ++i) DT<T>::st(next_in + e + i, f[i]); }
        }
    }
}

template <typename T, int NC>
__global__ __launch_bounds__(256) void sample_pred_wave_kernel(const DecodeState* st, const T* logits, int V, int cb,
                                                              SampleCfg c_imm, const T* noise_imm, int* codes, int G,
                                                              int64_t* out64, const T* next_emb, T* next_in, int H, const TeacherForcing* tf) {
    sample_pred_wave_body<T, NC>(st, logits, V, cb, c_imm, noise_imm, codes, G, out64, next_emb, next_in, H, tf);
}

template <typename T, int NC, bool NUCLEUS = false>
__device__ __forceinline__ void sample_talker_wave_body(DecodeState* st, const T* logits, int V, const unsigned char* seen, int G,
                                                        const TeacherForcing* tf = nullptr) {
    __shared__ BlkSmem sm;
    Raw8<T> xraw[NC];
    issue_logits<T, NC>(xraw, logits, V);
    if (st->done) return;
    SampleCfg c;
    c.temperature = st->t_temperature; c.top_k = st->t_top_k; c.top_p = st->t_top_p; c.do_sample = st->t_do_sample;
    c.rep_penalty = st->t_rep_penalty;
    c.sup_lo = st->sup_lo; c.sup_hi = st->sup_hi; c.keep_id = st->eos_id;
    const int frame = st->frame;
    c.sup_extra = (frame + 1 < st->min_new) ? st->eos_id : -1;
    const T* noise = st->talker_noise
        ? gptr(reinterpret_cast<const T*>(st->talker_noise)) + (size_t)(frame % st->noise_frames) * V : nullptr;
    int tok;
    if constexpr (NUCLEUS) {
        __shared__ SampleSmem big;
        if (c.do_sample && c.top_p < 1.0f) tok = sample_nucleus_from_regs<T, NC>(xraw, V, c, seen, noise, big);
        else tok = sample_wave_core<T, NC>(xraw, V, c, seen, noise, sm);
    } else {
        tok = sample_wave_core<T, NC>(xraw, V, c, seen, noise, sm);
    }
    tok = forced_or(tf, (frame + 1) * G, tok);
    if (threadIdx.x == 0) { st->token = tok; st->frame = frame + 1; st->pos += 1; st->gen_step += 1; }
}
template <typename T, int NC>
__global__ __launch_bounds__(256) void sample_talker_wave_kernel(DecodeState* st, const T* logits, int V,
                                                                const unsigned char* seen, int G, const TeacherForcing* tf) {
    sample_talker_wave_body<T, NC>(st, logits, V, seen, G, tf);
}

}
```

Measured before the change: 36.69.

## Precompute per-token predictor layer-0 QKV table and add bounded top-k search

Builds a device table holding the first predictor layer's normed QKV projection for every codebook token (with the optional projection folded in), shared across contexts. The sampler copies the selected token's row into the qkv buffer, so later predictor passes skip the layer-0 QKV GEMV. It also adds selectable top-k search strategies in the wave sampler that narrow the radix bit range from the max/min keys and reuse the found max. The cost is a large one-time table build and extra device memory, plus bf16 rounding differences between the table and the live computation.

```diff
diff --git a/faster-qwen3-tts_amd/csrc/fq3_api.hip b/faster-qwen3-tts_amd/csrc/fq3_api.hip
--- a/faster-qwen3-tts_amd/csrc/fq3_api.hip
+++ b/faster-qwen3-tts_amd/csrc/fq3_api.hip
@@ -243,6 +243,7 @@
     return FQ3_OK;
 }
 
+static void pred_tab_release(fq3_ctx* c);
 extern "C" int fq3_set_option(fq3_ctx* c, const char* key, int value) {
     if (!c || !key) return fail(FQ3_EINVAL, "null argument");
     const std::string k(key);
@@ -256,6 +257,9 @@
     else if (k == "swiglu_tile") c->opt_swiglu_tile = value;
     else if (k == "packed_weights") c->opt_packed = value;
     else if (k == "skinny_gemm") c->opt_no_skinny = !value;
+    else if (k == "pred_qkv_table") c->opt_pred_tab = value;
+    else if (k == "pred_qkv_table_limit_mb") { pred_tab_release(c); c->pred_tab_limit_mb = value; }
+    else if (k == "sampler_search") c->opt_search = value;
     else return fail(FQ3_EINVAL, "unknown option: " + k);
     fq3_graph_reset(c);
     return FQ3_OK;
@@ -330,11 +334,100 @@
     return FQ3_OK;
 }
 
+template <typename T, int NCH, int PRO, int R>
+__global__ __launch_bounds__(256) void pred_qkv_build_kernel(GemvArgs a, size_t x_stride, size_t y_stride) {
+    a.x = reinterpret_cast<const T*>(a.x) + (size_t)blockIdx.y * x_stride;
+    a.y = reinterpret_cast<T*>(a.y) + (size_t)blockIdx.y * y_stride;
+    gemv_body<T, NCH, PRO, EPI_STORE, false, 1, R>(a);
+}
+template <int PRO>
+static int pred_qkv_build_launch(const GemvArgs& a, int rows, size_t xs, size_t ys, int rmax, hipStream_t s) {
+    using T = bf16_t;
+    const int need = (a.K + 511) / 512;
+    int R = (a.N + 1023) / 1024;
+    if (R > 2) R = 2;
+    if (rmax > 0 && R > rmax) R = rmax;
+    if (R < 1) R = 1;
+    const dim3 grid((a.N + 4 * R - 1) / (4 * R), rows);
+#define FQ3_TAB_LAUNCH(NCH) do { \
+        if (R == 2) hipLaunchKernelGGL((pred_qkv_build_kernel<T, NCH, PRO, 2>), grid, dim3(256), 0, s, a, xs, ys); \
+        else hipLaunchKernelGGL((pred_qkv_build_kernel<T, NCH, PRO, 1>), grid, dim3(256), 0, s, a, xs, ys); } while (0)
+    if (need <= 1) FQ3_TAB_LAUNCH(1);
+    else if (need <= 2) FQ3_TAB_LAUNCH(2);
+    else if (need <= 4) FQ3_TAB_LAUNCH(4);
+    else return FQ3_EUNSUPPORTED;
+#undef FQ3_TAB_LAUNCH
+    return FQ3_OK;
+}
+namespace {
+struct PredTabEntry { void* p; int refs; };
+std::mutex g_pred_tab_mu;
+std::map<std::vector<const void*>, PredTabEntry> g_pred_tab;
+}
+static void pred_tab_release(fq3_ctx* c) {
+    if (c->pred_tab) {
+        std::lock_guard<std::mutex> lk(g_pred_tab_mu);
+        auto it = g_pred_tab.find(c->pred_tab_key);
+        if (it != g_pred_tab.end() && --it->second.refs <= 0) {
+            (void)hipDeviceSynchronize();
+            (void)hipFree(it->second.p);
+            g_pred_tab.erase(it);
+        }
+    }
+    c->pred_tab = nullptr; c->pred_tab_tried = false; c->pred_tab_key.clear();
+}
+static void pred_tab_ensure(fq3_ctx* c, hipStream_t s) {
+    if (c->pred_tab || c->pred_tab_tried || !c->opt_pred_tab || c->cfg.dtype != FQ3_BF16) return;
+    hipStreamCaptureStatus cst = hipStreamCaptureStatusNone;
+    if (hipStreamIsCapturing(s, &cst) != hipSuccess) { (void)hipGetLastError(); return; }
+    if (cst != hipStreamCaptureStatusNone) return;
+    c->pred_tab_tried = true;
+    const fq3_stack_dims &p = c->cfg.predictor, &t = c->cfg.talker;
+    const int G = c->cfg.num_code_groups, n_cb = G - 2, Vp = p.vocab;
+    const int N = (p.n_heads + 2 * p.n_kv_heads) * kHeadDim;
+    if (n_cb < 1 || (!c->cfg.has_projection && t.hidden != p.hidden)) return;
+    const size_t bytes = (size_t)n_cb * Vp * N * 2;
+    if (c->pred_tab_limit_mb > 0 && bytes > ((size_t)c->pred_tab_limit_mb << 20)) return;
+    std::vector<const void*> key{c->pl[0].qkv, c->pl[0].input_norm, c->cfg.has_projection ? c->wt.proj_w : nullptr,
+                                 c->cfg.has_projection ? c->wt.proj_b : nullptr};
+    for (int cb = 0; cb < n_cb; ++cb) key.push_back(c->pemb[cb]);
+    std::lock_guard<std::mutex> lk(g_pred_tab_mu);
+    auto it = g_pred_tab.find(key);
+    if (it != g_pred_tab.end()) { ++it->second.refs; c->pred_tab = it->second.p; c->pred_tab_key = key; return; }
+    void *tab = nullptr, *proj = nullptr;
+    hipStream_t bs = nullptr;
+    bool ok = hipMalloc(&tab, bytes) == hipSuccess;
+    if (ok && c->cfg.has_projection) ok = hipMalloc(&proj, (size_t)Vp * p.hidden * 2) == hipSuccess;
+    if (ok) ok = hipStreamCreateWithFlags(&bs, hipStreamNonBlocking) == hipSuccess;
+    if (ok) ok = hipStreamSynchronize(s) == hipSuccess;
+    for (int cb = 0; ok && cb < n_cb; ++cb) {
+        const void* x = c->pemb[cb];
+        size_t xs = (size_t)t.hidden;
+        if (c->cfg.has_projection) {
+            GemvArgs g{};
+            g.W = c->wt.proj_w; g.bias = c->wt.proj_b; g.N = p.hidden; g.K = t.hidden; g.x = x; g.y = proj;
+            ok = pred_qkv_build_launch<PRO_PLAIN>(g, Vp, xs, (size_t)p.hidden, c->opt_rmax, bs) == FQ3_OK;
+            x = proj; xs = (size_t)p.hidden;
+        }
+        GemvArgs g{};
+        g.eps = p.rms_eps; g.W = c->pl[0].qkv; g.N = N; g.K = p.hidden; g.x = x; g.norm_w = c->pl[0].input_norm;
+        g.y = reinterpret_cast<bf16_t*>(tab) + (size_t)cb * Vp * N;
+        if (ok) ok = pred_qkv_build_launch<PRO_NORM>(g, Vp, xs, (size_t)N, c->opt_rmax, bs) == FQ3_OK;
+    }
+    if (ok) ok = hipGetLastError() == hipSuccess && hipStreamSynchronize(bs) == hipSuccess;
+    if (bs) (void)hipStreamDestroy(bs);
+    if (proj) (void)hipFree(proj);
+    if (!ok) { (void)hipGetLastError(); if (tab) (void)hipFree(tab); return; }
+    g_pred_tab[key] = PredTabEntry{tab, 1};
+    c->pred_tab = tab; c->pred_tab_key = key;
+}
+
 extern "C" int fq3_ctx_destroy(fq3_ctx* c) {
     if (!c) return FQ3_OK;
     (void)hipDeviceSynchronize();
     fq3_graph_reset(c);
     packed_release_all(c);
+    pred_tab_release(c);
     if (c->cap_stream) (void)hipStreamDestroy(c->cap_stream);
     if (fq3_kv_pool* p = c->tk.pool) {
         (void)fq3_kv_release(c, 0);
@@ -369,6 +462,7 @@
     HIPCHK(hipMemcpy(c->d_pemb, c->pemb.data(), (G - 1) * sizeof(void*), hipMemcpyHostToDevice));
     (void)hipDeviceSynchronize();
     packed_release_all(c);
+    pred_tab_release(c);
     if (int r = packed_acquire_all(c)) { packed_release_all(c); return r; }
     c->bound = true;
     fq3_graph_reset(c);
@@ -437,7 +531,8 @@
     if (a.table) launch_attn_p<T, true>(a, rep, workers, s); else launch_attn_p<T, false>(a, rep, workers, s);
 }
 
-struct StepSrc { const void* x0; const int* pos_ptr; int pos_imm; bool kv_only_tail = false; };
+struct StepSrc { const void* x0; const int* pos_ptr; int pos_imm; bool kv_only_tail = false;
+                 bool qkv0_ready = false; };
 
 static int run_stack(fq3_ctx* c, bool talker, const StepSrc& src, hipStream_t s) {
     const fq3_stack_dims& d = talker ? c->cfg.talker : c->cfg.predictor;
@@ -462,7 +557,8 @@
         g.eps = d.rms_eps;
         g.W = w.qkv; g.N = q_dim + 2 * kv_dim; g.K = d.hidden; g.x = xin;
         g.norm_w = w.input_norm; g.y = c->qkv;
-        if (int r = launch_gemv<PRO_NORM, EPI_STORE>(c, g, nt, s)) return r;
+        if (!(i == 0 && src.qkv0_ready))
+            if (int r = launch_gemv<PRO_NORM, EPI_STORE>(c, g, nt, s)) return r;
         const bool tail_skip = src.kv_only_tail && i == d.n_layers - 1;
         GemvArgs o{};
         o.W = w.o; o.N = d.hidden; o.K = q_dim; o.y = c->h; o.res = xin; o.rep = rep;
@@ -801,21 +897,21 @@
 template <typename T>
 static void launch_sample_pred(const DecodeState* st, const T* lg, int V, int cb, const SampleCfg& cfg, const T* nz,
                                int* codes, int G, int64_t* out64, const T* next_emb, T* next_in, int H, bool wave,
-                               const TeacherForcing* tf, hipStream_t s) {
+                               const TeacherForcing* tf, const PredQkvRow<T>& qt, int search, hipStream_t s) {
     if (wave) dispatch_nc(V, [&](auto nc) {
         constexpr int NC = decltype(nc)::value;
         hipLaunchKernelGGL((sample_pred_wave_kernel<T, NC>), dim3(1), dim3(256), 0, s, st, lg, V, cb, cfg, nz, codes, G,
-                           out64, next_emb, next_in, H, tf);
+                           out64, next_emb, next_in, H, tf, qt, search);
     });
     else hipLaunchKernelGGL((sample_pred_kernel<T>), dim3(1), dim3(256), 0, s, st, lg, V, cb, cfg, nz, codes, G, out64,
-                            next_emb, next_in, H, tf);
+                            next_emb, next_in, H, tf, qt);
 }
 template <typename T>
 static void launch_sample_talker(DecodeState* st, const T* lg, int V, const unsigned char* seen, int G, bool wave,
-                                 const TeacherForcing* tf, hipStream_t s) {
+                                 const TeacherForcing* tf, int search, hipStream_t s) {
     if (wave) dispatch_nc(V, [&](auto nc) {
         constexpr int NC = decltype(nc)::value;
-        hipLaunchKernelGGL((sample_talker_wave_kernel<T, NC>), dim3(1), dim3(256), 0, s, st, lg, V, seen, G, tf);
+        hipLaunchKernelGGL((sample_talker_wave_kernel<T, NC>), dim3(1), dim3(256), 0, s, st, lg, V, seen, G, tf, search);
     });
     else hipLaunchKernelGGL((sample_talker_kernel<T>), dim3(1), dim3(256), 0, s, st, lg, V, seen, G, tf);
 }
@@ -830,7 +926,7 @@
         }
         dispatch_nc(V, [&](auto nc) {
             constexpr int NC = decltype(nc)::value;
-            hipLaunchKernelGGL((sample_api_wave_kernel<T, NC>), dim3(1), dim3(256), 0, s, lg, V, cfg, seen, noise, out);
+            hipLaunchKernelGGL((sample_api_wave_kernel<T, NC>), dim3(1), dim3(256), 0, s, lg, V, cfg, seen, noise, out, c->opt_search);
         });
     } else {
         hipLaunchKernelGGL((sample_api_kernel<T>), dim3(1), dim3(256), 0, s, lg, V, cfg, history, n_hist, noise, out);
@@ -898,6 +994,8 @@
     const fq3_stack_dims &p = c->cfg.predictor, &t = c->cfg.talker;
     const int G = c->cfg.num_code_groups, Vp = p.vocab, Ht = t.hidden;
     SampleCfg scfg = to_cfg(c->pred_sampling);
+    const T* qkv_tab = c->opt_pred_tab && sizeof(T) == 2 ? (const T*)c->pred_tab : nullptr;
+    const int qkv_n = (p.n_heads + 2 * p.n_kv_heads) * kHeadDim;
     for (int pass = 0; pass < G; ++pass) {
         const void* hsrc = c->h;
         if (pass == 0 && c->opt_m2) {
@@ -923,6 +1021,7 @@
         }
         StepSrc src{x0, nullptr, pass};
         src.kv_only_tail = pass == 0;
+        src.qkv0_ready = qkv_tab && pass >= 2;
         if (int r = run_stack(c, false, src, s)) return r;
         }
         if (pass == 0) continue;
@@ -934,8 +1033,10 @@
         if (int r = launch_gemv<PRO_NORM, EPI_STORE>(c, hgm, false, s)) return r;
         const T* nz = noise_imm ? (const T*)noise_imm + (size_t)cb * Vp : nullptr;
         const T* next_emb = cb + 1 < G - 1 ? (const T*)c->pemb[cb] : nullptr;
+        PredQkvRow<T> qt{};
+        if (qkv_tab && next_emb) { qt.tab = qkv_tab + (size_t)cb * Vp * qkv_n; qt.out = (T*)c->qkv; qt.n = qkv_n; qt.rows = Vp; }
         launch_sample_pred<T>(st_dev, (const T*)lg, Vp, cb, scfg, nz, st_dev ? c->codes : nullptr, G, out64, next_emb,
-                              (T*)c->pred_next, Ht, c->pred_sampling.top_p >= 1.0f, st_dev ? c->tf : nullptr, s);
+                              (T*)c->pred_next, Ht, c->pred_sampling.top_p >= 1.0f, st_dev ? c->tf : nullptr, qt, c->opt_search, s);
     }
     return 0;
 }
@@ -946,9 +1047,47 @@
     if (!pred_input || !out_ids) return fail(FQ3_EINVAL, "null argument");
     if (c->pred_sampling.do_sample && !noise) return fail(FQ3_EINVAL, "predictor sampling enabled but no noise given");
     hipStream_t s = (hipStream_t)stream;
+    pred_tab_ensure(c, s);
     int r = c->cfg.dtype == FQ3_BF16 ? predictor_passes_t<bf16_t>(c, nullptr, pred_input, noise, out_ids, out_logits, s)
                                      : predictor_passes_t<float>(c, nullptr, pred_input, noise, out_ids, out_logits, s);
     if (r) return r;
+    LAUNCH_CHECK();
+    return FQ3_OK;
+}
+
+extern "C" int64_t fq3_pred_qkv_table_bytes_(fq3_ctx* c, void* stream) {
+    if (!c || !c->bound) return 0;
+    pred_tab_ensure(c, (hipStream_t)stream);
+    if (!c->pred_tab || !c->opt_pred_tab) return 0;
+    const fq3_stack_dims& p = c->cfg.predictor;
+    return (int64_t)(c->cfg.num_code_groups - 2) * p.vocab * (p.n_heads + 2 * p.n_kv_heads) * kHeadDim * 2;
+}
+extern "C" int fq3_pred_qkv_table_probe_(fq3_ctx* c, int cb, const int* toks, int n, void* out_tab, void* out_live, void* stream) {
+    NEED_BOUND(c);
+    if (!toks || !out_tab || !out_live) return fail(FQ3_EINVAL, "null argument");
+    hipStream_t s = (hipStream_t)stream;
+    pred_tab_ensure(c, s);
+    if (!c->pred_tab) return fail(FQ3_ESTATE, "the context has no per-token qkv table");
+    const fq3_stack_dims &p = c->cfg.predictor, &t = c->cfg.talker;
+    if (cb < 0 || cb >= c->cfg.num_code_groups - 2) return fail(FQ3_EINVAL, "codebook outside the table");
+    const int N = (p.n_heads + 2 * p.n_kv_heads) * kHeadDim;
+    const bool nt = c->opt_nt == 2;
+    for (int i = 0; i < n; ++i) {
+        if (toks[i] < 0 || toks[i] >= p.vocab) return fail(FQ3_EINVAL, "token outside the predictor vocabulary");
+        const bf16_t* row = (const bf16_t*)c->pred_tab + ((size_t)cb * p.vocab + toks[i]) * N;
+        HIPCHK(hipMemcpyAsync((bf16_t*)out_tab + (size_t)i * N, row, (size_t)N * 2, hipMemcpyDeviceToDevice, s));
+        const void* x0 = (const bf16_t*)c->pemb[cb] + (size_t)toks[i] * t.hidden;
+        if (c->cfg.has_projection) {
+            GemvArgs g{};
+            g.W = c->wt.proj_w; g.bias = c->wt.proj_b; g.N = p.hidden; g.K = t.hidden; g.x = x0; g.y = c->pred_x;
+            if (int r = launch_gemv<PRO_PLAIN, EPI_STORE>(c, g, false, s)) return r;
+            x0 = c->pred_x;
+        }
+        GemvArgs g{};
+        g.eps = p.rms_eps; g.W = c->pl[0].qkv; g.N = N; g.K = p.hidden; g.x = x0; g.norm_w = c->pl[0].input_norm;
+        g.y = (bf16_t*)out_live + (size_t)i * N;
+        if (int r = launch_gemv<PRO_NORM, EPI_STORE>(c, g, nt, s)) return r;
+    }
     LAUNCH_CHECK();
     return FQ3_OK;
 }
@@ -977,6 +1116,7 @@
     const bool wave = p->talker.top_p >= 1.0f;
     if (wave != c->talker_wave) { fq3_graph_reset(c); c->talker_wave = wave; }
     hipStream_t s = (hipStream_t)stream;
+    pred_tab_ensure(c, s);
     if (int r = fq3_kv_ensure_(c, p->prefill_len + p->max_new_tokens + 1, s)) return r;
     DecodeState h{};
     h.token = p->first_token; h.frame = 0; h.pos = p->prefill_len; h.gen_step = p->gen_step; h.done = 0; h.text_open = 0;
@@ -1038,7 +1178,7 @@
     g.eps = t.rms_eps; g.W = c->wt.codec_head; g.N = t.vocab; g.K = H; g.x = c->h;
     g.norm_w = c->wt.talker_final_norm; g.y = c->logits; g.xn_out = c->past_hidden;
     if (int r = launch_gemv<PRO_NORM, EPI_STORE>(c, g, true, s)) return r;
-    launch_sample_talker<T>(st, (const T*)c->logits, t.vocab, c->seen, G, c->talker_wave, c->tf, s);
+    launch_sample_talker<T>(st, (const T*)c->logits, t.vocab, c->seen, G, c->talker_wave, c->tf, c->opt_search, s);
     return 0;
 }
 static int enqueue_frame(fq3_ctx* c, hipStream_t s) {
@@ -1048,7 +1188,7 @@
 extern "C" int fq3_graph_capture(fq3_ctx* c, void* stream) {
     NEED_BOUND(c);
     if (c->exec) return FQ3_OK;
-    (void)stream;
+    pred_tab_ensure(c, (hipStream_t)stream);
     hipStream_t cs = c->cap_stream;
     HIPCHK(hipStreamBeginCapture(cs, hipStreamCaptureModeRelaxed));
     int r = enqueue_frame(c, cs);
diff --git a/faster-qwen3-tts_amd/csrc/fq3_ctx.h b/faster-qwen3-tts_amd/csrc/fq3_ctx.h
--- a/faster-qwen3-tts_amd/csrc/fq3_ctx.h
+++ b/faster-qwen3-tts_amd/csrc/fq3_ctx.h
@@ -59,6 +59,12 @@
     int opt_swiglu_tile = 1;
     int opt_packed = 1;
     std::vector<std::pair<const void*, int>> packed_refs;
+    int opt_pred_tab = 1;
+    int opt_search = 0;
+    int pred_tab_limit_mb = 0;
+    const void* pred_tab = nullptr;
+    bool pred_tab_tried = false;
+    std::vector<const void*> pred_tab_key;
     int opt_no_skinny = 0;
     int prefill_mode = 0;
     bool talker_wave = true;
diff --git a/faster-qwen3-tts_amd/csrc/sampler.cuh b/faster-qwen3-tts_amd/csrc/sampler.cuh
--- a/faster-qwen3-tts_amd/csrc/sampler.cuh
+++ b/faster-qwen3-tts_amd/csrc/sampler.cuh
@@ -167,10 +167,21 @@
     if (threadIdx.x == 0) out[0] = tok;
 }
 
+template <typename T> struct PredQkvRow { const T* tab = nullptr; T* out = nullptr; int n = 0; int rows = 0; };
+template <typename T>
+__device__ __forceinline__ void pred_qkv_row_copy(const PredQkvRow<T>& q, int tok) {
+    if (!q.tab || (unsigned)tok >= (unsigned)q.rows) return;
+    constexpr int EPC = 16 / (int)sizeof(T);
+    const u32x4* src = reinterpret_cast<const u32x4*>(q.tab + (size_t)tok * q.n);
+    u32x4* dst = reinterpret_cast<u32x4*>(q.out);
+    for (int e = threadIdx.x; e < q.n / EPC; e += 256) dst[e] = src[e];
+}
+
 template <typename T>
 __global__ __launch_bounds__(256) void sample_pred_kernel(const DecodeState* st, const T* logits, int V, int cb,
                                                           SampleCfg c_imm, const T* noise_imm, int* codes, int G,
-                                                          int64_t* out64, const T* next_emb, T* next_in, int H, const TeacherForcing* tf) {
+                                                          int64_t* out64, const T* next_emb, T* next_in, int H, const TeacherForcing* tf,
+                                                          PredQkvRow<T> qt) {
     if (st && st->done) return;
     __shared__ SampleSmem sm;
     __shared__ int s_tok;
@@ -193,6 +204,7 @@
     }
     if (next_emb)
         for (int e = threadIdx.x; e < H; e += 256) next_in[e] = next_emb[(size_t)tok * H + e];
+    pred_qkv_row_copy(qt, tok);
 }
 
 template <typename T>
diff --git a/faster-qwen3-tts_amd/csrc/sampler_wave.cuh b/faster-qwen3-tts_amd/csrc/sampler_wave.cuh
--- a/faster-qwen3-tts_amd/csrc/sampler_wave.cuh
+++ b/faster-qwen3-tts_amd/csrc/sampler_wave.cuh
@@ -10,7 +10,18 @@
     return r;
 }
 
-struct BlkSmem { int cnt[2][4]; float f[4]; float av[4]; int ai[4]; };
+__device__ __forceinline__ int wave_max_i32(int v) {
+    v = max(v, dpp_move_i<kDppXor1, 0xF>(v, v)); v = max(v, dpp_move_i<kDppXor2, 0xF>(v, v));
+    v = max(v, dpp_move_i<kDppHalfMirror, 0xF>(v, v)); v = max(v, dpp_move_i<kDppMirror, 0xF>(v, v));
+    v = max(v, dpp_move_i<kDppBcast15, 0xA>(v, v));
+    v = max(v, dpp_move_i<kDppBcast31, 0xC>(v, v));
+    return __builtin_amdgcn_readlane(v, 63);
+}
+__device__ __forceinline__ float okey_inv(uint32_t k) { return __uint_as_float((k & 0x80000000u) ? (k & 0x7fffffffu) : ~k); }
+
+enum { SEARCH_BOUNDED = 0, SEARCH_FULL = 1 };
+
+struct BlkSmem { int cnt[2][4]; float f[4]; float av[4]; int ai[4]; int hi[4]; int lo[4]; };
 
 __device__ __forceinline__ float blk_max4(float v, BlkSmem& sm) {
     v = wave_max(v);
@@ -37,9 +48,9 @@
     return r.i;
 }
 
-template <typename T, int NC>
+template <typename T, int NC, bool WAVE0 = false>
 __device__ int sample_wave_core(Raw8<T> (&xraw)[NC], int V, const SampleCfg& c, const unsigned char* seen,
-                                const T* noise, BlkSmem& sm) {
+                                const T* noise, BlkSmem& sm, int search = SEARCH_BOUNDED) {
     const int tid = threadIdx.x;
     float x[NC][8];
     Raw8<T> nz[NC];
@@ -77,6 +88,8 @@
     for (int j = 0; j < NC; ++j)
 #pragma unroll
         for (int i = 0; i < 8; ++i) x[j][i] = DT<T>::rnd(x[j][i] / c.temperature);
+    uint32_t kmax = 0;
+    const bool have_kmax = c.top_k > 0 && (WAVE0 || search == SEARCH_BOUNDED);
     if (c.top_k > 0) {
         const int kk = min(c.top_k, V);
         uint32_t key[NC][8];
@@ -87,8 +100,67 @@
         uint32_t prefix = 0;
         constexpr int kLowBit = sizeof(T) == 2 ? 16 : 0;
         const int wave = tid >> 6;
+        int bit0 = 31;
+        if constexpr (WAVE0) {
+            __shared__ uint32_t skeys[NC * 2048];
+#pragma unroll
+            for (int j = 0; j < NC; ++j) {
+                u32x4* d = reinterpret_cast<u32x4*>(skeys + j * 2048 + tid * 8);
+                d[0] = u32x4{key[j][0], key[j][1], key[j][2], key[j][3]};
+                d[1] = u32x4{key[j][4], key[j][5], key[j][6], key[j][7]};
+            }
+            __syncthreads();
+            if (wave == 0) {
+                uint32_t wk[NC * 32];
+                uint32_t tm = 0;
+#pragma unroll
+                for (int t = 0; t < NC * 32; ++t) { wk[t] = skeys[t * 64 + tid]; tm = max(tm, wk[t]); }
+                const int ts = (int)(tm ^ 0x80000000u);
+                const uint32_t m = (uint32_t)wave_max_i32(ts) ^ 0x80000000u, lb = (uint32_t)wave_min_i32(ts) ^ 0x80000000u;
+                int b0 = 31;
+                uint32_t pf = 0;
+                if (kk <= 64 && lb > okey(-INFINITY)) {
+                    const uint32_t diff = m ^ lb;
+                    b0 = diff ? 31 - __clz(diff) : kLowBit - 1;
+                    if (b0 < kLowBit - 1) b0 = kLowBit - 1;
+                    pf = b0 >= 31 ? 0u : (m & ~((1u << (b0 + 1)) - 1u));
+                }
 #pragma unroll 1
-        for (int bit = 31; bit >= kLowBit; --bit) {
+                for (int bit = b0; bit >= kLowBit; --bit) {
+                    const uint32_t cand = pf | (1u << bit);
+                    int cnt = 0;
+#pragma unroll
+                    for (int t = 0; t < NC * 32; ++t) cnt += wk[t] >= cand ? 1 : 0;
+                    const int tot = wave_sum_i32(cnt);
+                    if (tot >= kk) pf = cand;
+                    if (tot == kk) break;
+                }
+                if (tid == 0) { sm.hi[0] = (int)pf; sm.hi[1] = (int)m; }
+            }
+            __syncthreads();
+            prefix = (uint32_t)sm.hi[0]; kmax = (uint32_t)sm.hi[1];
+            bit0 = kLowBit - 1;
+        } else if (search == SEARCH_BOUNDED) {
+            uint32_t tm = key[0][0];
+#pragma unroll
+            for (int j = 0; j < NC; ++j)
+#pragma unroll
+                for (int i = 0; i < 8; ++i) tm = max(tm, key[j][i]);
+            const int ts = (int)(tm ^ 0x80000000u);
+            const int whi = wave_max_i32(ts), wlo = wave_min_i32(ts);
+            if ((tid & 63) == 0) { sm.hi[wave] = whi; sm.lo[wave] = wlo; }
+            __syncthreads();
+            kmax = (uint32_t)max(max(sm.hi[0], sm.hi[1]), max(sm.hi[2], sm.hi[3])) ^ 0x80000000u;
+            const uint32_t lb = (uint32_t)min(min(sm.lo[0], sm.lo[1]), min(sm.lo[2], sm.lo[3])) ^ 0x80000000u;
+            if (kk <= 256 && lb > okey(-INFINITY)) {
+                const uint32_t diff = kmax ^ lb;
+                bit0 = diff ? 31 - __clz(diff) : kLowBit - 1;
+                if (bit0 < kLowBit - 1) bit0 = kLowBit - 1;
+                prefix = bit0 >= 31 ? 0u : (kmax & ~((1u << (bit0 + 1)) - 1u));
+            }
+        }
+#pragma unroll 1
+        for (int bit = bit0; bit >= kLowBit; --bit) {
             const uint32_t cand = prefix | (1u << bit);
             int cnt = 0;
 #pragma unroll
@@ -108,12 +180,16 @@
             for (int i = 0; i < 8; ++i)
                 if (key[j][i] < prefix) x[j][i] = -INFINITY;
     }
-    float mx = -INFINITY;
-#pragma unroll
-    for (int j = 0; j < NC; ++j)
-#pragma unroll
-        for (int i = 0; i < 8; ++i) mx = fmaxf(mx, x[j][i]);
-    mx = blk_max4(mx, sm);
+    float mx;
+    if (have_kmax) mx = okey_inv(kmax);
+    else {
+        mx = -INFINITY;
+#pragma unroll
+        for (int j = 0; j < NC; ++j)
+#pragma unroll
+            for (int i = 0; i < 8; ++i) mx = fmaxf(mx, x[j][i]);
+        mx = blk_max4(mx, sm);
+    }
     float se = 0.f;
 #pragma unroll
     for (int j = 0; j < NC; ++j)
@@ -147,11 +223,21 @@
 
 template <typename T, int NC>
 __global__ __launch_bounds__(256) void sample_api_wave_kernel(const T* logits, int V, SampleCfg c, const unsigned char* seen,
-                                                             const T* noise, int64_t* out) {
+                                                             const T* noise, int64_t* out, int search) {
     __shared__ BlkSmem sm;
     Raw8<T> xraw[NC];
     issue_logits<T, NC>(xraw, logits, V);
-    const int tok = sample_wave_core<T, NC>(xraw, V, c, seen, noise, sm);
+    const int tok = sample_wave_core<T, NC>(xraw, V, c, seen, noise, sm, search);
+    if (threadIdx.x == 0) out[0] = tok;
+}
+
+template <typename T, int NC>
+__global__ __launch_bounds__(256) void sample_api_wave0_kernel(const T* logits, int V, SampleCfg c, const unsigned char* seen,
+                                                              const T* noise, int64_t* out) {
+    __shared__ BlkSmem sm;
+    Raw8<T> xraw[NC];
+    issue_logits<T, NC>(xraw, logits, V);
+    const int tok = sample_wave_core<T, NC, true>(xraw, V, c, seen, noise, sm);
     if (threadIdx.x == 0) out[0] = tok;
 }
 
@@ -177,7 +263,8 @@
 template <typename T, int NC, bool NUCLEUS = false>
 __device__ __forceinline__ void sample_pred_wave_body(const DecodeState* st, const T* logits, int V, int cb,
                                                       const SampleCfg& c_imm, const T* noise_imm, int* codes, int G,
-                                                      int64_t* out64, const T* next_emb, T* next_in, int H, const TeacherForcing* tf = nullptr) {
+                                                      int64_t* out64, const T* next_emb, T* next_in, int H, const TeacherForcing* tf = nullptr,
+                                                      const PredQkvRow<T>& qt = PredQkvRow<T>{}, int search = SEARCH_BOUNDED) {
     __shared__ BlkSmem sm;
     Raw8<T> xraw[NC];
     issue_logits<T, NC>(xraw, logits, V);
@@ -195,9 +282,9 @@
     if constexpr (NUCLEUS) {
         __shared__ SampleSmem big;
         if (c.do_sample && c.top_p < 1.0f) tok = sample_nucleus_from_regs<T, NC>(xraw, V, c, nullptr, noise, big);
-        else tok = sample_wave_core<T, NC>(xraw, V, c, nullptr, noise, sm);
+        else tok = sample_wave_core<T, NC>(xraw, V, c, nullptr, noise, sm, search);
     } else {
-        tok = sample_wave_core<T, NC>(xraw, V, c, nullptr, noise, sm);
+        tok = sample_wave_core<T, NC>(xraw, V, c, nullptr, noise, sm, search);
     }
     if (st) tok = forced_or(tf, frame * G + 1 + cb, tok);
     if (threadIdx.x == 0) {
@@ -214,18 +301,20 @@
                    for (int i = 0; i < 8; ++i) DT<T>::st(next_in + e + i, f[i]); }
         }
     }
+    pred_qkv_row_copy(qt, tok);
 }
 
 template <typename T, int NC>
 __global__ __launch_bounds__(256) void sample_pred_wave_kernel(const DecodeState* st, const T* logits, int V, int cb,
                                                               SampleCfg c_imm, const T* noise_imm, int* codes, int G,
-                                                              int64_t* out64, const T* next_emb, T* next_in, int H, const TeacherForcing* tf) {
-    sample_pred_wave_body<T, NC>(st, logits, V, cb, c_imm, noise_imm, codes, G, out64, next_emb, next_in, H, tf);
+                                                              int64_t* out64, const T* next_emb, T* next_in, int H, const TeacherForcing* tf,
+                                                              PredQkvRow<T> qt, int search) {
+    sample_pred_wave_body<T, NC>(st, logits, V, cb, c_imm, noise_imm, codes, G, out64, next_emb, next_in, H, tf, qt, search);
 }
 
 template <typename T, int NC, bool NUCLEUS = false>
 __device__ __forceinline__ void sample_talker_wave_body(DecodeState* st, const T* logits, int V, const unsigned char* seen, int G,
-                                                        const TeacherForcing* tf = nullptr) {
+                                                        const TeacherForcing* tf = nullptr, int search = SEARCH_BOUNDED) {
     __shared__ BlkSmem sm;
     Raw8<T> xraw[NC];
     issue_logits<T, NC>(xraw, logits, V);
@@ -242,17 +331,17 @@
     if constexpr (NUCLEUS) {
         __shared__ SampleSmem big;
         if (c.do_sample && c.top_p < 1.0f) tok = sample_nucleus_from_regs<T, NC>(xraw, V, c, seen, noise, big);
-        else tok = sample_wave_core<T, NC>(xraw, V, c, seen, noise, sm);
+        else tok = sample_wave_core<T, NC>(xraw, V, c, seen, noise, sm, search);
     } else {
-        tok = sample_wave_core<T, NC>(xraw, V, c, seen, noise, sm);
+        tok = sample_wave_core<T, NC>(xraw, V, c, seen, noise, sm, search);
     }
     tok = forced_or(tf, (frame + 1) * G, tok);
     if (threadIdx.x == 0) { st->token = tok; st->frame = frame + 1; st->pos += 1; st->gen_step += 1; }
 }
 template <typename T, int NC>
 __global__ __launch_bounds__(256) void sample_talker_wave_kernel(DecodeState* st, const T* logits, int V,
-                                                                const unsigned char* seen, int G, const TeacherForcing* tf) {
-    sample_talker_wave_body<T, NC>(st, logits, V, seen, G, tf);
-}
-
-}
+                                                                const unsigned char* seen, int G, const TeacherForcing* tf, int search) {
+    sample_talker_wave_body<T, NC>(st, logits, V, seen, G, tf, search);
+}
+
+}
```

New measurement: 36.60. No clear change (-0.2%).
